# Samsung/iac

Measured on AMD Instinct MI355X. Metric: Msamples/s rendered (3rd-order HOA->binaural, 48 kHz), higher is better.
Workload: dtype f32

## Files before the change

### iac_amd/csrc/iamf_render.hip

```cpp
#include <hip/hip_runtime.h>

#include <math.h>
#include <stdint.h>
#include <atomic>
#include <stdio.h>
#include <stdlib.h>
#include <string.h>

#include <new>
#include <type_traits>
#include <vector>

#include "../../include/iamf_hip.h"

#define IAMF_FFT_HOST_TABLES

#include "render_entry.hpp"

namespace {

#include "render_common.hpp"
#include "render_downmix.hpp"
#include "render_fir.hpp"
#include "render_fir16.hpp"
// ... 46 lines not shown
};

extern "C" const uint8_t _binary_rdr_tables_bin_start[];
extern "C" const uint8_t _binary_rdr_tables_bin_end[];
extern "C" const uint8_t _binary_rdr_tables_tv_bin_start[];
extern "C" const uint8_t _binary_rdr_tables_tv_bin_end[];

struct Tables {
  int n = 0;
  const TableEntry *ents = nullptr;
  const float *data = nullptr;
  bool ok = false;
  explicit Tables(bool tv) {
    const uint8_t *b = tv ? _binary_rdr_tables_tv_bin_start : _binary_rdr_tables_bin_start;
    const size_t sz = tv ? (size_t)(_binary_rdr_tables_tv_bin_end - _binary_rdr_tables_tv_bin_start)
                         : (size_t)(_binary_rdr_tables_bin_end - _binary_rdr_tables_bin_start);
    if (sz < 12 || memcmp(b, "IARDRTB1", 8) != 0) return;
    uint32_t cnt;
    memcpy(&cnt, b + 8, 4);
    n = (int)cnt;
    ents = reinterpret_cast<const TableEntry *>(b + 12);
    data = reinterpret_cast<const float *>(b + 12 + sizeof(TableEntry) * cnt);
    ok = true;
  }
};

const Tables &tables(bool tv) {
  static Tables t(false), t_tv(true);
  return tv ? t_tv : t;
}

int find_matrix(int kind, int in_id, int out_id, iamf_hip_matrix *out, bool tv = false) {
  const Tables &t = tables(tv);
  if (!t.ok || !out) return -1;
  for (int i = 0; i < t.n; ++i) {
    const TableEntry &e = t.ents[i];
    if ((int)e.kind == kind && (int)e.in_id == in_id && (int)e.out_id == out_id) {
      out->kind = kind;
      out->in_id = in_id;
      out->out_id = out_id;
      out->channels = e.channels;
      out->lfe1 = e.lfe1;
      out->lfe2 = e.lfe2;
      out->m = e.m;
      out->n = e.n;
      out->mat = t.data + e.offset;
      return 0;
    }
  }
  return -1;
}

float ease(float x) {
  if (1.0 < x) return 1.0f;
  if (x < 0) return 0.0f;
  return 1.0f - powf(x - 1, 2.0);
}

}

struct iamf_hip_batch {
  iamf_hip_batch_config cfg;
  int device = 0;
  hipEvent_t done = nullptr;
  bool rendered = false;
  int m = 0, n_feeds = 0;
  int32_t src_feed[kMaxOut];
  uint32_t nz_mask[6] = {0, 0, 0, 0, 0, 0};
  int sparse = 0;
  int32_t *d_src_feed = nullptr;
  float thr = 0.f;
  int n_atk = 0, n_end = 0;
  std::vector<int64_t> spos;
  std::vector<uint8_t> sflushed;
  bool any_rendered = false;
  bool lp_scale_ok = false;
  float *d_matrix = nullptr, *d_gains = nullptr, *d_ctab = nullptr, *d_ring_y = nullptr,
        *d_ring_pm = nullptr;
  LimState *d_lim = nullptr;
  std::vector<float> h_gains;
  bool has2 = false;
  int m2 = 0;
  float *d_matrix2 = nullptr, *d_gains2 = nullptr;
  int32_t *d_src_feed2 = nullptr, *d_dmx_tab = nullptr;
  bool dmx = false;
  int dmx_n_in = 0, dmx_n_out = 0;
  float *d_pre = nullptr;
  int pre_l = 0;
  std::vector<float> h_fm;
  float *d_matrix_pre = nullptr;
  uint32_t nz_mask_pre[6] = {0, 0, 0, 0, 0, 0};
  int sparse_pre = 0;
  bool demix = false;
  int demix_steps = 0, demix_skip = 0, demix_layout = 0, demix_gmask = 0, demix_w4 = 0;
  int32_t *d_demix_tab = nullptr;
  float *d_demix_ftab = nullptr;
  bool fir = false;
  int fir_taps = 0;
  float *d_fir_hist[2] = {nullptr, nullptr};
  void *d_fir_h16 = nullptr;
  float *d_fir_pq = nullptr, *d_fir_tw = nullptr;
  float *d_fir_zero = nullptr;
  float *d_fir_pre[2] = {nullptr, nullptr};
  size_t fir_pre_bytes = 0;
  float *d_fir_y = nullptr;
  size_t fir_y_floats = 0;
  float *d_lp_in = nullptr;
  size_t lp_in_floats = 0;
  float *d_fir_id = nullptr;
  int32_t *d_fir_id_feed = nullptr;
  float fir_inv_scale = 1.f;
  int fir_cur = 0;
  bool lfe = false;
  float lfe_a1 = 0.f, lfe_a2 = 0.f, lfe_a3 = 0.f, lfe_b1 = 0.f, lfe_b2 = 0.f;
  double lfe_div = 0.0;
  float *d_lfe_state = nullptr, *d_lfe_next = nullptr, *d_lfe_u = nullptr;
  bool lfe_shared = false;
  size_t lfe_u_floats = 0;
  uint8_t *d_nat = nullptr;
  size_t nat_bytes = 0;
  uint8_t *d_dump = nullptr;
};

namespace {

bool on_batch_device(const iamf_hip_batch *b) {
  int dev = -1;
  return hipGetDevice(&dev) == hipSuccess && dev == b->device;
}

int quiesce(iamf_hip_batch *b) {
  if (b->rendered) HIPCHK(hipEventSynchronize(b->done));
  return IAMF_HIP_OK;
}

int reset_state(iamf_hip_batch *b) {
  const int ns = b->cfg.n_streams;
  std::vector<LimState> init((size_t)ns);
  for (auto &l : init) {
    l.g = 1.0f;
    l.gs = -1.0f;
    l.ge = -1.0f;
    l.n = b->n_end;
  }
  HIPCHK(hipMemcpy(b->d_lim, init.data(), sizeof(LimState) * ns, hipMemcpyHostToDevice));
  HIPCHK(hipMemset(b->d_ring_y, 0, sizeof(float) * (size_t)ns * b->cfg.out_channels * kSave));
  HIPCHK(hipMemset(b->d_ring_pm, 0, sizeof(float) * (size_t)ns * kSave));
  if (b->fir) {
    const size_t hb = sizeof(float) * (size_t)ns * b->m * 256;
    HIPCHK(hipMemset(b->d_fir_hist[0], 0, hb));
    HIPCHK(hipMemset(b->d_fir_hist[1], 0, hb));
    for (float *q : b->d_fir_pre)
      if (q) HIPCHK(hipMemset(q, 0, b->fir_pre_bytes));
  }
  if (b->lfe && !b->lfe_shared) {
    HIPCHK(hipMemset(b->d_lfe_state, 0, sizeof(float) * 4 * (size_t)ns));
    HIPCHK(hipMemset(b->d_lfe_next, 0, sizeof(float) * 2 * (size_t)ns));
  }
  b->spos.assign((size_t)ns, 0);
  b->sflushed.assign((size_t)ns, 0);
  b->any_rendered = false;
  return IAMF_HIP_OK;
}

template <int M>
void launch_m(const RenderParams &p, dim3 grid, size_t lds_bytes, hipStream_t st) {
  hipLaunchKernelGGL(render_kernel<M>, grid, dim3(kChunk), lds_bytes, st, p);
}

template <int M>
void launch_nolim_m(const RenderParams &p, hipStream_t st) {
  const int bytes = p.out_format == IAMF_HIP_FMT_S16 ? 2 : (p.out_format == IAMF_HIP_FMT_S24 ? 3 : 4);
  dim3 grid((unsigned)p.n_launch, (unsigned)((p.total + kNlChunk - 1) / kNlChunk));
  hipLaunchKernelGGL(render_nolim_kernel<M>, grid, dim3(256), (size_t)kNlChunk * p.out_ch * bytes, st, p);
}

template <int M, int OC>
void launch_fast_mc(const RenderParams &p, bool mixing, dim3 grid, hipStream_t st) {
  const size_t lds = sizeof(float) * (size_t)fast_lds_floats(OC, M);
  if (mixing) launch_big_lds<&render_fast_kernel<M, OC, 0, false, true>, 80 * 1024>(grid, dim3(256), lds, st, p);
  else launch_big_lds<&render_fast_kernel<M, OC>, 80 * 1024>(grid, dim3(256), lds, st, p);
}
template <int M>
void launch_fast_m(const RenderParams &p, bool mixing, dim3 grid, hipStream_t st) {
  if (p.out_ch == 1) launch_fast_mc<M, 1>(p, mixing, grid, st);
  else launch_fast_mc<M, 2>(p, mixing, grid, st);
}

template <int M, int OC>
void launch_fast_down_mc(const RenderParams &p, dim3 grid, hipStream_t st) {
  const size_t lds = sizeof(float) * (size_t)fast_lds_floats(OC, M);
  launch_big_lds<&render_fast_kernel<M, OC, 0, true>, 80 * 1024>(grid, dim3(256), lds, st, p);
}

template <int M>
void launch_wide_m(const RenderParams &p, dim3 grid, hipStream_t st) {
  const size_t lds = sizeof(float) * (size_t)wide_lds_floats(p.out_ch, M);
  if (p.use_mfma) launch_big_lds<&render_wide_kernel<M, true>, 80 * 1024>(grid, dim3(256), lds, st, p);
  else launch_big_lds<&render_wide_kernel<M, false>, 80 * 1024>(grid, dim3(256), lds, st, p);
}

int launch(const RenderParams &p, int m, size_t lds_bytes, hipStream_t st) {
  const Route r = pick_route(p, m);
  const dim3 grid((unsigned)p.n_launch);
  bool launched = false;
  switch (r.family) {
    case Family::Refused: return r.err;
    case Family::Lpcm: launched = iamf_hip_fast_lpcm_launch(&p, m, r.variant, st); break;
    case Family::FirSplit: {
      if (!dispatch(FirHomeM{}, m, [&](auto M) { launch_fft_m<M.value>(p, st); }) && !iamf_hip_fir_m2b_launch_fft(&p, m, st))
        return IAMF_HIP_ERR_INTERNAL;
      HIPCHK(hipGetLastError());
      RenderParams q = p;
      q.in = p.fir_y;
      q.in_stream_stride = 2 * (int64_t)p.total;
      q.in_frame_stride = 2 * (int64_t)p.total;
      q.frame_size = p.total;
      q.matrix = p.fir_id_matrix;
      q.src_feed = p.fir_id_feed;
      q.n_feeds = 2;
      q.fir_taps = 0;
      q.fir_hist = q.fir_hist_next = nullptr;
      launch_fast_m<2>(q, false, grid, st);
      launched = true;
      break;
    }
    case Family::FirFused:
      launched = dispatch(FirHomeM{}, m, [&](auto M) { launch_fir_m<M.value>(p, r.variant, st); }) ||
                 iamf_hip_fir_m2b_launch(&p, m, r.variant, st);
      break;
    case Family::FastDown:
      launched = dispatch(FastDownMC{}, mc(m, p.out_ch), [&](auto V) { launch_fast_down_mc<mc_m(V.value), mc_c(V.value)>(p, grid, st); });
      break;
    case Family::Wide4Lfe: launched = iamf_hip_wide4_lfe_launch(&p, m, st); break;
    case Family::Wide4Mix: launched = iamf_hip_wide4_mix_launch(&p, m, st); break;
    case Family::Wide4:
    case Family::Wide4Demix:
    case Family::Wide4Down: launched = iamf_hip_wide4_launch(&p, m, st); break;
    case Family::Nolim: launched = dispatch(NolimM{}, m, [&](auto M) { launch_nolim_m<M.value>(p, st); }); break;
    case Family::Fast: launched = dispatch(FastM{}, m, [&](auto M) { launch_fast_m<M.value>(p, r.variant != 0, grid, st); }); break;
    case Family::Wide: launched = dispatch(WideM{}, m, [&](auto M) { launch_wide_m<M.value>(p, grid, st); }); break;
    case Family::Generic: launched = dispatch(GenericM{}, m, [&](auto M) { launch_m<M.value>(p, grid, lds_bytes, st); }); break;
  }
  if (!launched) return IAMF_HIP_ERR_INTERNAL;
  HIPCHK(hipGetLastError());
  const RouteKey k = route_key(r, p, m);
  iamf_hip_route_count(k.family, k.variant, k.m, k.c, k.k);
  if (r.family == Family::FirSplit) iamf_hip_route_count(IAMF_HIP_ROUTE_FAST, 0, 2, 2, 0);
  return IAMF_HIP_OK;
}

const int kLayoutCount[9] = {1, 2, 6, 8, 10, 8, 10, 12, 6};
const int kLayoutCh[9][12] = {
    {kChMono},
    {kChL2, kChR2},
    {kChL7, kChR7, kChC, kChLFE, kChSL5, kChSR5},
    {kChL7, kChR7, kChC, kChLFE, kChSL5, kChSR5, kChHL, kChHR},
    {kChL7, kChR7, kChC, kChLFE, kChSL5, kChSR5, kChHFL, kChHFR, kChHBL, kChHBR},
    {kChL7, kChR7, kChC, kChLFE, kChSL7, kChSR7, kChBL7, kChBR7},
    {kChL7, kChR7, kChC, kChLFE, kChSL7, kChSR7, kChBL7, kChBR7, kChHL, kChHR},
    {kChL7, kChR7, kChC, kChLFE, kChSL7, kChSR7, kChBL7, kChBR7, kChHFL, kChHFR, kChHBL, kChHBR},
    {kChL3, kChR3, kChC, kChLFE, kChTL, kChTR},
};
const int kLayoutSurround[9] = {1, 2, 5, 5, 5, 7, 7, 7, 3};
const int kLayoutTop[9] = {0, 0, 0, 2, 4, 0, 2, 4, 2};

struct LpcmIn {
  const uint8_t *raw;
  int64_t stream_stride, frame_stride;
  int32_t off[16];
};
constexpr int kNotFused = INT32_MIN;

int lfe_prepass(iamf_hip_batch *b, const float *d_in, int64_t in_stream_stride, int64_t in_frame_stride, int ltotal,
                hipStream_t st, int s0, int cnt, int *t4_out) {
  const int ns = b->cfg.n_streams, nb = (ns + 63) / 64, t4 = (ltotal + 3) / 4;
  const size_t need_u = (size_t)nb * t4 * 64 * 4;
  if (need_u > b->lfe_u_floats) {
    HIPCHK(hipStreamSynchronize(st));
    (void)hipFree(b->d_lfe_u);
    b->d_lfe_u = nullptr;
    b->lfe_u_floats = 0;
    HIPCHK(hipMalloc(&b->d_lfe_u, sizeof(float) * need_u));
    b->lfe_u_floats = need_u;
  }
  LfeParams lp;
  memset(&lp, 0, sizeof(lp));
  lp.in = d_in;
  lp.in_stream_stride = in_stream_stride;
  lp.in_frame_stride = in_frame_stride;
  lp.pre_matrix = b->d_pre;
  lp.pre_l = b->pre_l;
  lp.pre_m = b->m;
  lp.frame_size = b->cfg.frame_size;
  lp.n_streams = ns;
  lp.total = ltotal;
  lp.t4 = t4;
  lp.a1 = b->lfe_a1; lp.a2 = b->lfe_a2; lp.a3 = b->lfe_a3; lp.b1 = b->lfe_b1; lp.b2 = b->lfe_b2;
  lp.state = b->d_lfe_state;
  lp.state_next = b->d_lfe_next;
  lp.u_t = reinterpret_cast<float4 *>(b->d_lfe_u);
  lp.s_first = s0;
  lp.s_count = cnt;
  hipLaunchKernelGGL(lfe_ff_kernel, dim3((unsigned)((t4 + kLfeTileQ - 1) / kLfeTileQ), (unsigned)nb), dim3(256), 0, st, lp);
  hipLaunchKernelGGL(lfe_chain_kernel, dim3((unsigned)nb), dim3(64), 0, st, lp);
  HIPCHK(hipGetLastError());
  *t4_out = t4;
  return IAMF_HIP_OK;
}

struct PreparedCall {
  RenderParams p;
  iamf_hip_render_args a;
  int m_eff;
  size_t lds;
  bool restride;
  int sc, bps;
  int64_t pos;
  int total, s0, cnt;
};

int render_prepare(iamf_hip_batch *b, const iamf_hip_render_args &a, int total, int s0, int cnt, const LpcmIn *lp, PreparedCall &pc) {
  if (!on_batch_device(b)) return IAMF_HIP_ERR_INVALID_STATE;
  if (lp && (b->fir || b->lfe || b->d_pre || b->demix || b->dmx || b->has2 || a.d_element_ramp || a.d_element2_ramp ||
             a.d_output_ramp || !b->lp_scale_ok || getenv("IAMF_HIP_LPCM_UNFUSED")))
    return kNotFused;
  if (s0 < 0 || cnt <= 0 || s0 + cnt > b->cfg.n_streams) return IAMF_HIP_ERR_BAD_ARG;
  if (a.lfe_pre_samples < 0 || a.lfe_post_samples < 0 ||
      ((a.lfe_pre_samples || a.lfe_post_samples) &&
       (a.n_frames != 1 || (int64_t)a.lfe_pre_samples + total + a.lfe_post_samples > b->cfg.frame_size)))
    return IAMF_HIP_ERR_BAD_ARG;
  const int64_t pos = b->spos[(size_t)s0];
  for (int i = s0; i < s0 + cnt; ++i)
    if (b->spos[(size_t)i] != pos || b->sflushed[(size_t)i]) return IAMF_HIP_ERR_INVALID_STATE;
  const bool whole = s0 == 0 && cnt == b->cfg.n_streams;
  if (!whole && b->fir) return IAMF_HIP_ERR_UNIMPLEMENTED;
  RenderParams &p = pc.p;
  memset(&p, 0, sizeof(p));
  p.stream0 = s0;
  p.n_launch = cnt;
  p.in = a.d_in;
  p.in_stream_stride = a.in_stream_stride;
  p.in_frame_stride = a.in_frame_stride;
  p.pcm = static_cast<uint8_t *>(a.d_pcm);
  p.pcm_stream_stride = a.pcm_stream_stride_bytes;
  p.matrix = b->d_matrix;
  p.gains = b->d_gains;
  p.ctab = b->d_ctab;
  p.lim = b->d_lim;
  p.ring_y = b->d_ring_y;
  p.ring_pm = b->d_ring_pm;
  p.pos0 = pos;
  p.total = total;
  p.frame_size = b->cfg.frame_size;
  p.n_streams = b->cfg.n_streams;
  p.n_feeds = b->n_feeds;
  p.out_ch = b->cfg.out_channels;
  p.og_ch = (b->cfg.out_gain_channels > 0 && b->cfg.out_gain_channels < b->cfg.out_channels) ? b->cfg.out_gain_channels : b->cfg.out_channels;
  p.out_format = b->cfg.out_format;
  p.limiter_on = b->cfg.limiter_enable ? 1 : 0;
  p.loudness_on = b->cfg.loudness_enable ? 1 : 0;
  bool tolerance = false;
  {
    const int proj = b->cfg.projection;
    const char *env = getenv("IAMF_HIP_PROJECTION");
    bool mf = proj == IAMF_HIP_PROJ_MFMA || (proj == IAMF_HIP_PROJ_AUTO && b->cfg.matrix.kind == IAMF_HIP_KIND_H2M);
    if (env && !strcmp(env, "exact")) mf = false;
    if (env && !strcmp(env, "mfma")) mf = true;
    p.use_mfma = (mf && b->n_feeds <= 32) ? 1 : 0;
    tolerance = mf;
  }
  p.n_atk = b->n_atk;
  p.n_end = b->n_end;
  p.thr = b->thr;
  p.src_feed = b->d_src_feed;
  p.dump = b->d_dump;
  for (int g = 0; g < 6; ++g) p.nz_mask[g] = b->nz_mask[g];
  p.sparse = getenv("IAMF_HIP_DENSE") ? 0 : b->sparse;
  if (b->has2 && a.d_in2) {
    p.in2 = a.d_in2;
    p.in2_stream_stride = a.in2_stream_stride;
    p.in2_frame_stride = a.in2_frame_stride;
    p.matrix2 = b->d_matrix2;
    p.src_feed2 = b->d_src_feed2;
    p.gains2 = b->d_gains2;
    p.m2 = b->m2;
  }
  p.elem_ramp = a.d_element_ramp;
  p.elem2_ramp = a.d_element2_ramp;
  p.out_ramp = a.d_output_ramp;
  p.ramp_stream_stride = a.ramp_stream_stride;
  if (b->dmx) {
    p.dmx_on = 1;
    p.dmx_frames = a.d_in ? a.d_dmx_frames : nullptr;
    p.dmx_n_in = b->dmx_n_in;
    p.dmx_n_out = b->dmx_n_out;
    p.dmx_tab = b->d_dmx_tab;
    p.dmx_in_layout = b->cfg.matrix.in_id;
    p.dmx_out_layout = b->cfg.matrix.out_id;
  }
  int m_eff = b->m;
  if (b->d_pre && a.d_in) {
    const int l = b->pre_l;
    if (tolerance && b->d_matrix_pre && FastM::has(l) && !p.in2) {
      p.matrix = b->d_matrix_pre;
      for (int g = 0; g < 6; ++g) p.nz_mask[g] = b->nz_mask_pre[g];
      p.sparse = getenv("IAMF_HIP_DENSE") ? 0 : b->sparse_pre;
      m_eff = l;
    } else {
      p.pre_matrix = b->d_pre;
      p.pre_l = b->pre_l;
    }
  }
  if (b->demix && a.d_in) {
    p.demix_on = 1;
    p.demix_steps = b->demix_steps;
    p.demix_skip = b->demix_skip;
    p.demix_tab = b->d_demix_tab;
    p.demix_ftab = b->d_demix_ftab;
    p.demix_frames = a.d_demix_frames;
    p.demix_i0 = a.n_frames == 1 ? a.demix_sample0 : 0;
    p.demix_layout = b->demix_layout;
    p.demix_gmask = b->demix_gmask;
    p.demix_w4 = b->demix_w4;
  }
  if (lp) {
    p.lpcm = lp->raw;
    p.lpcm_stream_stride = lp->stream_stride;
    p.lpcm_frame_stride = lp->frame_stride;
    for (int m = 0; m < 16; ++m) p.lpcm_off[m] = lp->off[m];
    if (pick_route(p, m_eff).family != Family::Lpcm) return kNotFused;
  }
  if (b->fir) {
    p.fir_taps = b->fir_taps;
    p.fir_hist = b->d_fir_hist[b->fir_cur];
    p.fir_hist_next = b->d_fir_hist[b->fir_cur ^ 1];
    p.fir_h16 = b->d_fir_h16;
    p.fir_inv_scale = b->fir_inv_scale;
    p.fir_pq = b->d_fir_pq;
    p.fir_tw = b->d_fir_tw;
    p.fir_zero = b->d_fir_zero;
    p.fir_pre = b->d_fir_pre[b->fir_cur];
    p.fir_pre_next = b->d_fir_pre[b->fir_cur ^ 1];
    if (a.d_in && b->d_fir_pq && (b->cfg.frame_size & 63) == 0 && !getenv("IAMF_HIP_FIR_FUSED") && !getenv("IAMF_HIP_FIR_F16") &&
        !getenv("IAMF_HIP_FIR_F32")) {
      const size_t need = (size_t)b->cfg.n_streams * 2 * (size_t)total;
      if (need > b->fir_y_floats) {
        HIPCHK(hipStreamSynchronize(static_cast<hipStream_t>(a.stream)));
        (void)hipFree(b->d_fir_y);
        b->d_fir_y = nullptr;
        b->fir_y_floats = 0;
        HIPCHK(hipMalloc(&b->d_fir_y, sizeof(float) * need));
        b->fir_y_floats = need;
      }
      p.fir_y = b->d_fir_y;
      p.fir_id_matrix = b->d_fir_id;
      p.fir_id_feed = b->d_fir_id_feed;
    }
  }
  if (b->lfe && a.d_in && total > 0) {
    const int lpre = a.lfe_pre_samples, lpost = a.lfe_post_samples;
    int t4 = 0;
    const int rc = lfe_prepass(b, a.d_in - lpre, a.in_stream_stride, a.in_frame_stride, lpre + total + lpost,
                               static_cast<hipStream_t>(a.stream), s0, cnt, &t4);
    if (rc) return rc;
    p.lfe = b->d_lfe_u;
    p.lfe_t4 = t4;
    p.lfe_k0 = lpre;
    p.lfe_div = b->lfe_div;
    for (int c = 0; c < b->cfg.out_channels && c < 32; ++c)
      if (b->src_feed[c] == -2) p.lfe_mask |= 1 << c;
  }
  const size_t lds = sizeof(float) * ((size_t)(p.out_ch + 2) * kRing + 3 * kChunk + kHead + 4 +
                                      ((b->dmx || b->demix) ? (size_t)kChCount * kChunk : 0));
  const int sc = b->cfg.pcm_stride_channels;
  const bool restride = sc > 0 && sc != p.out_ch;
  const int bps = iamf_hip_format_bytes(p.out_format);
  if (restride) {
    const size_t per_stream = (size_t)(total > kDelay ? total : kDelay) * p.out_ch * bps;
    const size_t need = per_stream * (size_t)p.n_streams;
    if (need > b->nat_bytes) {
      HIPCHK(hipStreamSynchronize(static_cast<hipStream_t>(a.stream)));
      (void)hipFree(b->d_nat);
      b->d_nat = nullptr;
      b->nat_bytes = 0;
      HIPCHK(hipMalloc(&b->d_nat, need));
      b->nat_bytes = need;
    }
    p.pcm = b->d_nat;
    p.pcm_stream_stride = (int64_t)per_stream;
  }
  pc.a = a;
  pc.m_eff = m_eff;
  pc.lds = lds;
  pc.restride = restride;
  pc.sc = sc;
  pc.bps = bps;
  pc.pos = pos;
  pc.total = total;
  pc.s0 = s0;
  pc.cnt = cnt;
  return IAMF_HIP_OK;
}

int render_launch(const PreparedCall &pc) {
  return launch(pc.p, pc.m_eff, pc.lds, static_cast<hipStream_t>(pc.a.stream));
}

int render_commit(iamf_hip_batch *b, const PreparedCall &pc) {
  const RenderParams &p = pc.p;
  const iamf_hip_render_args &a = pc.a;
  const bool restride = pc.restride;
  const int sc = pc.sc, bps = pc.bps, total = pc.total, s0 = pc.s0, cnt = pc.cnt;
  const int64_t pos = pc.pos;
  if (b->fir && p.in) b->fir_cur ^= 1;
  const int64_t before = p.limiter_on ? (pos > kDelay ? pos - kDelay : 0) : pos;
  for (int i = s0; i < s0 + cnt; ++i) b->spos[(size_t)i] = pos + total;
  b->any_rendered = true;
  const int64_t after = p.limiter_on ? (pos + total > kDelay ? pos + total - kDelay : 0) : pos + total;
  const int n_emit = (int)(after - before);
  if (restride && n_emit > 0) {
    const int64_t n_out = (int64_t)n_emit * sc + (p.out_ch > sc ? p.out_ch - sc : 0);
    hipLaunchKernelGGL(restride_kernel, dim3((unsigned)((n_out + 255) / 256), (unsigned)cnt), dim3(256), 0,
                       static_cast<hipStream_t>(a.stream), b->d_nat, p.pcm_stream_stride,
                       static_cast<uint8_t *>(a.d_pcm), a.pcm_stream_stride_bytes, n_emit, p.out_ch, sc, bps, s0);
    HIPCHK(hipGetLastError());
  }
  HIPCHK(hipEventRecord(b->done, static_cast<hipStream_t>(a.stream)));
  b->rendered = true;
  return n_emit;
}

int render_call(iamf_hip_batch *b, const iamf_hip_render_args &a, int total, int s0, int cnt, const LpcmIn *lp = nullptr) {
  PreparedCall pc;
  int r = render_prepare(b, a, total, s0, cnt, lp, pc);
  if (r != IAMF_HIP_OK) return r;
  r = render_launch(pc);
  if (r != IAMF_HIP_OK) return r;
  return render_commit(b, pc);
}

void build_feed_map(const iamf_hip_matrix &mx, int out_channels, std::vector<float> &fm, int32_t *src_feed) {
  for (int i = 0; i < kMaxOut; ++i) src_feed[i] = -1;
  for (int i = 0; i < mx.n; ++i) {
    int d = i;
    if (mx.kind == IAMF_HIP_KIND_H2M && (mx.lfe1 >= 0 || mx.lfe2 >= 0)) {
      if (mx.lfe1 >= 0 && mx.lfe1 <= i) ++d;
      if (mx.lfe2 >= 0 && mx.lfe2 <= i) ++d;
    }
    if (d < out_channels) src_feed[d] = i;
  }
  if (mx.kind == IAMF_HIP_KIND_H2M) {
    if (mx.lfe1 >= 0 && mx.lfe1 < out_channels) src_feed[mx.lfe1] = -1;
    if (mx.lfe2 >= 0 && mx.lfe2 < out_channels) src_feed[mx.lfe2] = -1;
  }
  fm.assign((size_t)mx.m * mx.n, 0.f);
  for (int f = 0; f < mx.n; ++f)
    for (int k = 0; k < mx.m; ++k)
      fm[(size_t)f * mx.m + k] = mx.kind == IAMF_HIP_KIND_H2M ? mx.mat[f * mx.m + k] : mx.mat[k * mx.n + f];
}

}

extern "C" {

int iamf_hip_get_h2m_matrix(int order, int out_id, iamf_hip_matrix *out) {
  return find_matrix(IAMF_HIP_KIND_H2M, order, out_id, out);
}

int iamf_hip_get_m2m_matrix(int in_id, int out_id, iamf_hip_matrix *out) {
  return find_matrix(IAMF_HIP_KIND_M2M, in_id, out_id, out);
}

int iamf_hip_get_m2m_matrix_variant(int variant, int in_id, int out_id, iamf_hip_matrix *out) {
  if (variant != IAMF_HIP_VARIANT_DEFAULT && variant != IAMF_HIP_VARIANT_SAMSUNG_TV) return -1;
  return find_matrix(IAMF_HIP_KIND_M2M, in_id, out_id, out, variant == IAMF_HIP_VARIANT_SAMSUNG_TV);
}

int iamf_hip_layout_channels(int out_id) {
  switch (out_id) {
    case IAMF_HIP_SS_A: return 2;
    case IAMF_HIP_SS_B: return 6;
    case IAMF_HIP_SS_C: return 8;
    case IAMF_HIP_SS_D: return 10;
    case IAMF_HIP_SS_E: return 11;
    case IAMF_HIP_SS_F: return 12;
    case IAMF_HIP_SS_G: return 14;
    case IAMF_HIP_SS_H: return 24;
    case IAMF_HIP_SS_I: return 8;
    case IAMF_HIP_SS_J: return 12;
    case IAMF_HIP_L_712: return 10;
    case IAMF_HIP_L_312: return 6;
    case IAMF_HIP_L_MONO: return 1;
    case IAMF_HIP_L_BINAURAL: return 2;
    default: return 0;
  }
}

int iamf_hip_format_bytes(int f) {
  switch (f) {
    case IAMF_HIP_FMT_S16: return 2;
    case IAMF_HIP_FMT_S24: return 3;
    case IAMF_HIP_FMT_S32: return 4;
    case IAMF_HIP_FMT_F32: return 4;
    default: return 0;
  }
}

// ... 1280 lines not shown
```

### iac_amd/csrc/lfe_chain_asm.inc

```
#define IAMF_LFE_RING 32
#define IAMF_LFE_ASM_BODY \
  "s_mov_b64 s[40:41], %[base]\n\t" \
  "s_mov_b32 s44, %[nrot]\n\t" \
  "v_mov_b32 v0, %[voff]\n\t" \
  "v_mov_b32 v2, %[b1]\n\t" \
  "v_mov_b32 v3, %[b2]\n\t" \
  "v_mov_b32 v12, 0x80000000\n\t" \
  "v_mov_b32 v13, 0x80000000\n\t" \
  "v_mul_f32 v10, v2, %[y1]\n\t" \
  "v_mul_f32 v11, v3, %[y1]\n\t" \
  "v_mul_f32 v9, v3, %[y2]\n\t" \
  "s_add_u32 s46, s40, 4096\n\t" \
  "s_addc_u32 s47, s41, 0\n\t" \
  "global_load_dwordx4 v[16:19], v0, s[46:47] offset:-4096\n\t" \
  "global_load_dwordx4 v[20:23], v0, s[46:47] offset:-3072\n\t" \
  "global_load_dwordx4 v[24:27], v0, s[46:47] offset:-2048\n\t" \
  "global_load_dwordx4 v[28:31], v0, s[46:47] offset:-1024\n\t" \
  "global_load_dwordx4 v[32:35], v0, s[46:47] offset:0\n\t" \
  "global_load_dwordx4 v[36:39], v0, s[46:47] offset:1024\n\t" \
  "global_load_dwordx4 v[40:43], v0, s[46:47] offset:2048\n\t" \
  "global_load_dwordx4 v[44:47], v0, s[46:47] offset:3072\n\t" \
  "s_add_u32 s46, s46, 8192\n\t" \
  "s_addc_u32 s47, s47, 0\n\t" \
  "global_load_dwordx4 v[48:51], v0, s[46:47] offset:-4096\n\t" \
  "global_load_dwordx4 v[52:55], v0, s[46:47] offset:-3072\n\t" \
  "global_load_dwordx4 v[56:59], v0, s[46:47] offset:-2048\n\t" \
  "global_load_dwordx4 v[60:63], v0, s[46:47] offset:-1024\n\t" \
  "global_load_dwordx4 v[64:67], v0, s[46:47] offset:0\n\t" \
  "global_load_dwordx4 v[68:71], v0, s[46:47] offset:1024\n\t" \
  "global_load_dwordx4 v[72:75], v0, s[46:47] offset:2048\n\t" \
  "global_load_dwordx4 v[76:79], v0, s[46:47] offset:3072\n\t" \
  "s_add_u32 s46, s46, 8192\n\t" \
  "s_addc_u32 s47, s47, 0\n\t" \
  "global_load_dwordx4 v[80:83], v0, s[46:47] offset:-4096\n\t" \
  "global_load_dwordx4 v[84:87], v0, s[46:47] offset:-3072\n\t" \
  "global_load_dwordx4 v[88:91], v0, s[46:47] offset:-2048\n\t" \
  "global_load_dwordx4 v[92:95], v0, s[46:47] offset:-1024\n\t" \
  "global_load_dwordx4 v[96:99], v0, s[46:47] offset:0\n\t" \
  "global_load_dwordx4 v[100:103], v0, s[46:47] offset:1024\n\t" \
  "global_load_dwordx4 v[104:107], v0, s[46:47] offset:2048\n\t" \
  "global_load_dwordx4 v[108:111], v0, s[46:47] offset:3072\n\t" \
  "s_add_u32 s46, s46, 8192\n\t" \
  "s_addc_u32 s47, s47, 0\n\t" \
  "global_load_dwordx4 v[112:115], v0, s[46:47] offset:-4096\n\t" \
  "global_load_dwordx4 v[116:119], v0, s[46:47] offset:-3072\n\t" \
  "global_load_dwordx4 v[120:123], v0, s[46:47] offset:-2048\n\t" \
  "global_load_dwordx4 v[124:127], v0, s[46:47] offset:-1024\n\t" \
  "global_load_dwordx4 v[128:131], v0, s[46:47] offset:0\n\t" \
  "global_load_dwordx4 v[132:135], v0, s[46:47] offset:1024\n\t" \
  "global_load_dwordx4 v[136:139], v0, s[46:47] offset:2048\n\t" \
  "global_load_dwordx4 v[140:143], v0, s[46:47] offset:3072\n\t" \
  "s_add_u32 s46, s46, 8192\n\t" \
  "s_addc_u32 s47, s47, 0\n\t" \
  "s_waitcnt vmcnt(0)\n\t" \
  "Llfe_rot%=:\n\t" \
  "s_sub_u32 s44, s44, 1\n\t" \
  "s_cmp_lg_u32 s44, 0\n\t" \
  "s_cselect_b32 s45, 32768, 0\n\t" \
  "s_add_u32 s42, s40, 4096\n\t" \
  "s_addc_u32 s43, s41, 0\n\t" \
  "s_add_u32 s46, s42, s45\n\t" \
  "s_addc_u32 s47, s43, 0\n\t" \
  "s_waitcnt vmcnt(56)\n\t" \
  "v_sub_f32 v16, v16, v10\n\t" \
  "v_sub_f32 v16, v16, v9\n\t" \
  "v_pk_mul_f32 v[4:5], v[16:17], v[2:3] op_sel:[0,0] op_sel_hi:[0,1]\n\t" \
  "v_sub_f32 v17, v17, v4\n\t" \
  "v_sub_f32 v17, v17, v11\n\t" \
  "v_pk_mul_f32 v[6:7], v[16:17], v[2:3] op_sel:[1,0] op_sel_hi:[1,1]\n\t" \
  "v_sub_f32 v18, v18, v6\n\t" \
  "v_sub_f32 v18, v18, v5\n\t" \
  "v_pk_mul_f32 v[8:9], v[18:19], v[2:3] op_sel:[0,0] op_sel_hi:[0,1]\n\t" \
  "v_sub_f32 v19, v19, v8\n\t" \
  "v_sub_f32 v19, v19, v7\n\t" \
  "v_pk_mul_f32 v[10:11], v[18:19], v[2:3] op_sel:[1,0] op_sel_hi:[1,1]\n\t" \
  "global_store_dwordx4 v0, v[16:19], s[42:43] offset:-4096\n\t" \
  "global_load_dwordx4 v[16:19], v0, s[46:47] offset:-4096\n\t" \
  "v_sub_f32 v20, v20, v10\n\t" \
  "v_sub_f32 v20, v20, v9\n\t" \
  "v_pk_mul_f32 v[4:5], v[20:21], v[2:3] op_sel:[0,0] op_sel_hi:[0,1]\n\t" \
  "v_sub_f32 v21, v21, v4\n\t" \
  "v_sub_f32 v21, v21, v11\n\t" \
  "v_pk_mul_f32 v[6:7], v[20:21], v[2:3] op_sel:[1,0] op_sel_hi:[1,1]\n\t" \
  "v_sub_f32 v22, v22, v6\n\t" \
  "v_sub_f32 v22, v22, v5\n\t" \
  "v_pk_mul_f32 v[8:9], v[22:23], v[2:3] op_sel:[0,0] op_sel_hi:[0,1]\n\t" \
  "v_sub_f32 v23, v23, v8\n\t" \
  "v_sub_f32 v23, v23, v7\n\t" \
  "v_pk_mul_f32 v[10:11], v[22:23], v[2:3] op_sel:[1,0] op_sel_hi:[1,1]\n\t" \
  "global_store_dwordx4 v0, v[20:23], s[42:43] offset:-3072\n\t" \
  "global_load_dwordx4 v[20:23], v0, s[46:47] offset:-3072\n\t" \
  "v_sub_f32 v24, v24, v10\n\t" \
  "v_sub_f32 v24, v24, v9\n\t" \
  "v_pk_mul_f32 v[4:5], v[24:25], v[2:3] op_sel:[0,0] op_sel_hi:[0,1]\n\t" \
  "v_sub_f32 v25, v25, v4\n\t" \
  "v_sub_f32 v25, v25, v11\n\t" \
  "v_pk_mul_f32 v[6:7], v[24:25], v[2:3] op_sel:[1,0] op_sel_hi:[1,1]\n\t" \
  "v_sub_f32 v26, v26, v6\n\t" \
  "v_sub_f32 v26, v26, v5\n\t" \
  "v_pk_mul_f32 v[8:9], v[26:27], v[2:3] op_sel:[0,0] op_sel_hi:[0,1]\n\t" \
  "v_sub_f32 v27, v27, v8\n\t" \
  "v_sub_f32 v27, v27, v7\n\t" \
  "v_pk_mul_f32 v[10:11], v[26:27], v[2:3] op_sel:[1,0] op_sel_hi:[1,1]\n\t" \
  "global_store_dwordx4 v0, v[24:27], s[42:43] offset:-2048\n\t" \
  "global_load_dwordx4 v[24:27], v0, s[46:47] offset:-2048\n\t" \
  "v_sub_f32 v28, v28, v10\n\t" \
  "v_sub_f32 v28, v28, v9\n\t" \
  "v_pk_mul_f32 v[4:5], v[28:29], v[2:3] op_sel:[0,0] op_sel_hi:[0,1]\n\t" \
  "v_sub_f32 v29, v29, v4\n\t" \
  "v_sub_f32 v29, v29, v11\n\t" \
  "v_pk_mul_f32 v[6:7], v[28:29], v[2:3] op_sel:[1,0] op_sel_hi:[1,1]\n\t" \
  "v_sub_f32 v30, v30, v6\n\t" \
  "v_sub_f32 v30, v30, v5\n\t" \
  "v_pk_mul_f32 v[8:9], v[30:31], v[2:3] op_sel:[0,0] op_sel_hi:[0,1]\n\t" \
  "v_sub_f32 v31, v31, v8\n\t" \
  "v_sub_f32 v31, v31, v7\n\t" \
  "v_pk_mul_f32 v[10:11], v[30:31], v[2:3] op_sel:[1,0] op_sel_hi:[1,1]\n\t" \
  "global_store_dwordx4 v0, v[28:31], s[42:43] offset:-1024\n\t" \
  "global_load_dwordx4 v[28:31], v0, s[46:47] offset:-1024\n\t" \
  "s_waitcnt vmcnt(56)\n\t" \
  "v_sub_f32 v32, v32, v10\n\t" \
  "v_sub_f32 v32, v32, v9\n\t" \
  "v_pk_mul_f32 v[4:5], v[32:33], v[2:3] op_sel:[0,0] op_sel_hi:[0,1]\n\t" \
  "v_sub_f32 v33, v33, v4\n\t" \
  "v_sub_f32 v33, v33, v11\n\t" \
  "v_pk_mul_f32 v[6:7], v[32:33], v[2:3] op_sel:[1,0] op_sel_hi:[1,1]\n\t" \
  "v_sub_f32 v34, v34, v6\n\t" \
  "v_sub_f32 v34, v34, v5\n\t" \
  "v_pk_mul_f32 v[8:9], v[34:35], v[2:3] op_sel:[0,0] op_sel_hi:[0,1]\n\t" \
  "v_sub_f32 v35, v35, v8\n\t" \
  "v_sub_f32 v35, v35, v7\n\t" \
  "v_pk_mul_f32 v[10:11], v[34:35], v[2:3] op_sel:[1,0] op_sel_hi:[1,1]\n\t" \
  "global_store_dwordx4 v0, v[32:35], s[42:43] offset:0\n\t" \
  "global_load_dwordx4 v[32:35], v0, s[46:47] offset:0\n\t" \
  "v_sub_f32 v36, v36, v10\n\t" \
  "v_sub_f32 v36, v36, v9\n\t" \
  "v_pk_mul_f32 v[4:5], v[36:37], v[2:3] op_sel:[0,0] op_sel_hi:[0,1]\n\t" \
  "v_sub_f32 v37, v37, v4\n\t" \
  "v_sub_f32 v37, v37, v11\n\t" \
  "v_pk_mul_f32 v[6:7], v[36:37], v[2:3] op_sel:[1,0] op_sel_hi:[1,1]\n\t" \
  "v_sub_f32 v38, v38, v6\n\t" \
  "v_sub_f32 v38, v38, v5\n\t" \
  "v_pk_mul_f32 v[8:9], v[38:39], v[2:3] op_sel:[0,0] op_sel_hi:[0,1]\n\t" \
  "v_sub_f32 v39, v39, v8\n\t" \
  "v_sub_f32 v39, v39, v7\n\t" \
  "v_pk_mul_f32 v[10:11], v[38:39], v[2:3] op_sel:[1,0] op_sel_hi:[1,1]\n\t" \
  "global_store_dwordx4 v0, v[36:39], s[42:43] offset:1024\n\t" \
  "global_load_dwordx4 v[36:39], v0, s[46:47] offset:1024\n\t" \
  "v_sub_f32 v40, v40, v10\n\t" \
  "v_sub_f32 v40, v40, v9\n\t" \
  "v_pk_mul_f32 v[4:5], v[40:41], v[2:3] op_sel:[0,0] op_sel_hi:[0,1]\n\t" \
  "v_sub_f32 v41, v41, v4\n\t" \
  "v_sub_f32 v41, v41, v11\n\t" \
  "v_pk_mul_f32 v[6:7], v[40:41], v[2:3] op_sel:[1,0] op_sel_hi:[1,1]\n\t" \
  "v_sub_f32 v42, v42, v6\n\t" \
  "v_sub_f32 v42, v42, v5\n\t" \
  "v_pk_mul_f32 v[8:9], v[42:43], v[2:3] op_sel:[0,0] op_sel_hi:[0,1]\n\t" \
  "v_sub_f32 v43, v43, v8\n\t" \
  "v_sub_f32 v43, v43, v7\n\t" \
  "v_pk_mul_f32 v[10:11], v[42:43], v[2:3] op_sel:[1,0] op_sel_hi:[1,1]\n\t" \
  "global_store_dwordx4 v0, v[40:43], s[42:43] offset:2048\n\t" \
  "global_load_dwordx4 v[40:43], v0, s[46:47] offset:2048\n\t" \
  "v_sub_f32 v44, v44, v10\n\t" \
  "v_sub_f32 v44, v44, v9\n\t" \
  "v_pk_mul_f32 v[4:5], v[44:45], v[2:3] op_sel:[0,0] op_sel_hi:[0,1]\n\t" \
  "v_sub_f32 v45, v45, v4\n\t" \
  "v_sub_f32 v45, v45, v11\n\t" \
  "v_pk_mul_f32 v[6:7], v[44:45], v[2:3] op_sel:[1,0] op_sel_hi:[1,1]\n\t" \
  "v_sub_f32 v46, v46, v6\n\t" \
  "v_sub_f32 v46, v46, v5\n\t" \
  "v_pk_mul_f32 v[8:9], v[46:47], v[2:3] op_sel:[0,0] op_sel_hi:[0,1]\n\t" \
  "v_sub_f32 v47, v47, v8\n\t" \
  "v_sub_f32 v47, v47, v7\n\t" \
  "v_pk_mul_f32 v[10:11], v[46:47], v[2:3] op_sel:[1,0] op_sel_hi:[1,1]\n\t" \
  "global_store_dwordx4 v0, v[44:47], s[42:43] offset:3072\n\t" \
  "global_load_dwordx4 v[44:47], v0, s[46:47] offset:3072\n\t" \
  "s_add_u32 s42, s42, 8192\n\t" \
  "s_addc_u32 s43, s43, 0\n\t" \
  "s_add_u32 s46, s46, 8192\n\t" \
  "s_addc_u32 s47, s47, 0\n\t" \
  "s_waitcnt vmcnt(56)\n\t" \
  "v_sub_f32 v48, v48, v10\n\t" \
  "v_sub_f32 v48, v48, v9\n\t" \
  "v_pk_mul_f32 v[4:5], v[48:49], v[2:3] op_sel:[0,0] op_sel_hi:[0,1]\n\t" \
  "v_sub_f32 v49, v49, v4\n\t" \
  "v_sub_f32 v49, v49, v11\n\t" \
  "v_pk_mul_f32 v[6:7], v[48:49], v[2:3] op_sel:[1,0] op_sel_hi:[1,1]\n\t" \
  "v_sub_f32 v50, v50, v6\n\t" \
  "v_sub_f32 v50, v50, v5\n\t" \
  "v_pk_mul_f32 v[8:9], v[50:51], v[2:3] op_sel:[0,0] op_sel_hi:[0,1]\n\t" \
  "v_sub_f32 v51, v51, v8\n\t" \
  "v_sub_f32 v51, v51, v7\n\t" \
  "v_pk_mul_f32 v[10:11], v[50:51], v[2:3] op_sel:[1,0] op_sel_hi:[1,1]\n\t" \
  "global_store_dwordx4 v0, v[48:51], s[42:43] offset:-4096\n\t" \
  "global_load_dwordx4 v[48:51], v0, s[46:47] offset:-4096\n\t" \
  "v_sub_f32 v52, v52, v10\n\t" \
  "v_sub_f32 v52, v52, v9\n\t" \
  "v_pk_mul_f32 v[4:5], v[52:53], v[2:3] op_sel:[0,0] op_sel_hi:[0,1]\n\t" \
  "v_sub_f32 v53, v53, v4\n\t" \
  "v_sub_f32 v53, v53, v11\n\t" \
  "v_pk_mul_f32 v[6:7], v[52:53], v[2:3] op_sel:[1,0] op_sel_hi:[1,1]\n\t" \
  "v_sub_f32 v54, v54, v6\n\t" \
  "v_sub_f32 v54, v54, v5\n\t" \
  "v_pk_mul_f32 v[8:9], v[54:55], v[2:3] op_sel:[0,0] op_sel_hi:[0,1]\n\t" \
  "v_sub_f32 v55, v55, v8\n\t" \
  "v_sub_f32 v55, v55, v7\n\t" \
  "v_pk_mul_f32 v[10:11], v[54:55], v[2:3] op_sel:[1,0] op_sel_hi:[1,1]\n\t" \
  "global_store_dwordx4 v0, v[52:55], s[42:43] offset:-3072\n\t" \
  "global_load_dwordx4 v[52:55], v0, s[46:47] offset:-3072\n\t" \
  "v_sub_f32 v56, v56, v10\n\t" \
  "v_sub_f32 v56, v56, v9\n\t" \
  "v_pk_mul_f32 v[4:5], v[56:57], v[2:3] op_sel:[0,0] op_sel_hi:[0,1]\n\t" \
  "v_sub_f32 v57, v57, v4\n\t" \
  "v_sub_f32 v57, v57, v11\n\t" \
  "v_pk_mul_f32 v[6:7], v[56:57], v[2:3] op_sel:[1,0] op_sel_hi:[1,1]\n\t" \
  "v_sub_f32 v58, v58, v6\n\t" \
  "v_sub_f32 v58, v58, v5\n\t" \
  "v_pk_mul_f32 v[8:9], v[58:59], v[2:3] op_sel:[0,0] op_sel_hi:[0,1]\n\t" \
  "v_sub_f32 v59, v59, v8\n\t" \
  "v_sub_f32 v59, v59, v7\n\t" \
  "v_pk_mul_f32 v[10:11], v[58:59], v[2:3] op_sel:[1,0] op_sel_hi:[1,1]\n\t" \
  "global_store_dwordx4 v0, v[56:59], s[42:43] offset:-2048\n\t" \
  "global_load_dwordx4 v[56:59], v0, s[46:47] offset:-2048\n\t" \
  "v_sub_f32 v60, v60, v10\n\t" \
  "v_sub_f32 v60, v60, v9\n\t" \
  "v_pk_mul_f32 v[4:5], v[60:61], v[2:3] op_sel:[0,0] op_sel_hi:[0,1]\n\t" \
  "v_sub_f32 v61, v61, v4\n\t" \
  "v_sub_f32 v61, v61, v11\n\t" \
  "v_pk_mul_f32 v[6:7], v[60:61], v[2:3] op_sel:[1,0] op_sel_hi:[1,1]\n\t" \
  "v_sub_f32 v62, v62, v6\n\t" \
  "v_sub_f32 v62, v62, v5\n\t" \
  "v_pk_mul_f32 v[8:9], v[62:63], v[2:3] op_sel:[0,0] op_sel_hi:[0,1]\n\t" \
  "v_sub_f32 v63, v63, v8\n\t" \
  "v_sub_f32 v63, v63, v7\n\t" \
  "v_pk_mul_f32 v[10:11], v[62:63], v[2:3] op_sel:[1,0] op_sel_hi:[1,1]\n\t" \
  "global_store_dwordx4 v0, v[60:63], s[42:43] offset:-1024\n\t" \
  "global_load_dwordx4 v[60:63], v0, s[46:47] offset:-1024\n\t" \
  "s_waitcnt vmcnt(56)\n\t" \
  "v_sub_f32 v64, v64, v10\n\t" \
  "v_sub_f32 v64, v64, v9\n\t" \
  "v_pk_mul_f32 v[4:5], v[64:65], v[2:3] op_sel:[0,0] op_sel_hi:[0,1]\n\t" \
  "v_sub_f32 v65, v65, v4\n\t" \
  "v_sub_f32 v65, v65, v11\n\t" \
  "v_pk_mul_f32 v[6:7], v[64:65], v[2:3] op_sel:[1,0] op_sel_hi:[1,1]\n\t" \
  "v_sub_f32 v66, v66, v6\n\t" \
  "v_sub_f32 v66, v66, v5\n\t" \
  "v_pk_mul_f32 v[8:9], v[66:67], v[2:3] op_sel:[0,0] op_sel_hi:[0,1]\n\t" \
  "v_sub_f32 v67, v67, v8\n\t" \
  "v_sub_f32 v67, v67, v7\n\t" \
  "v_pk_mul_f32 v[10:11], v[66:67], v[2:3] op_sel:[1,0] op_sel_hi:[1,1]\n\t" \
  "global_store_dwordx4 v0, v[64:67], s[42:43] offset:0\n\t" \
  "global_load_dwordx4 v[64:67], v0, s[46:47] offset:0\n\t" \
  "v_sub_f32 v68, v68, v10\n\t" \
  "v_sub_f32 v68, v68, v9\n\t" \
  "v_pk_mul_f32 v[4:5], v[68:69], v[2:3] op_sel:[0,0] op_sel_hi:[0,1]\n\t" \
  "v_sub_f32 v69, v69, v4\n\t" \
  "v_sub_f32 v69, v69, v11\n\t" \
  "v_pk_mul_f32 v[6:7], v[68:69], v[2:3] op_sel:[1,0] op_sel_hi:[1,1]\n\t" \
  "v_sub_f32 v70, v70, v6\n\t" \
  "v_sub_f32 v70, v70, v5\n\t" \
  "v_pk_mul_f32 v[8:9], v[70:71], v[2:3] op_sel:[0,0] op_sel_hi:[0,1]\n\t" \
  "v_sub_f32 v71, v71, v8\n\t" \
  "v_sub_f32 v71, v71, v7\n\t" \
  "v_pk_mul_f32 v[10:11], v[70:71], v[2:3] op_sel:[1,0] op_sel_hi:[1,1]\n\t" \
  "global_store_dwordx4 v0, v[68:71], s[42:43] offset:1024\n\t" \
  "global_load_dwordx4 v[68:71], v0, s[46:47] offset:1024\n\t" \
  "v_sub_f32 v72, v72, v10\n\t" \
  "v_sub_f32 v72, v72, v9\n\t" \
  "v_pk_mul_f32 v[4:5], v[72:73], v[2:3] op_sel:[0,0] op_sel_hi:[0,1]\n\t" \
  "v_sub_f32 v73, v73, v4\n\t" \
  "v_sub_f32 v73, v73, v11\n\t" \
  "v_pk_mul_f32 v[6:7], v[72:73], v[2:3] op_sel:[1,0] op_sel_hi:[1,1]\n\t" \
  "v_sub_f32 v74, v74, v6\n\t" \
  "v_sub_f32 v74, v74, v5\n\t" \
  "v_pk_mul_f32 v[8:9], v[74:75], v[2:3] op_sel:[0,0] op_sel_hi:[0,1]\n\t" \
  "v_sub_f32 v75, v75, v8\n\t" \
  "v_sub_f32 v75, v75, v7\n\t" \
  "v_pk_mul_f32 v[10:11], v[74:75], v[2:3] op_sel:[1,0] op_sel_hi:[1,1]\n\t" \
  "global_store_dwordx4 v0, v[72:75], s[42:43] offset:2048\n\t" \
  "global_load_dwordx4 v[72:75], v0, s[46:47] offset:2048\n\t" \
  "v_sub_f32 v76, v76, v10\n\t" \
  "v_sub_f32 v76, v76, v9\n\t" \
  "v_pk_mul_f32 v[4:5], v[76:77], v[2:3] op_sel:[0,0] op_sel_hi:[0,1]\n\t" \
  "v_sub_f32 v77, v77, v4\n\t" \
  "v_sub_f32 v77, v77, v11\n\t" \
  "v_pk_mul_f32 v[6:7], v[76:77], v[2:3] op_sel:[1,0] op_sel_hi:[1,1]\n\t" \
  "v_sub_f32 v78, v78, v6\n\t" \
  "v_sub_f32 v78, v78, v5\n\t" \
  "v_pk_mul_f32 v[8:9], v[78:79], v[2:3] op_sel:[0,0] op_sel_hi:[0,1]\n\t" \
  "v_sub_f32 v79, v79, v8\n\t" \
  "v_sub_f32 v79, v79, v7\n\t" \
  "v_pk_mul_f32 v[10:11], v[78:79], v[2:3] op_sel:[1,0] op_sel_hi:[1,1]\n\t" \
  "global_store_dwordx4 v0, v[76:79], s[42:43] offset:3072\n\t" \
  "global_load_dwordx4 v[76:79], v0, s[46:47] offset:3072\n\t" \
  "s_add_u32 s42, s42, 8192\n\t" \
  "s_addc_u32 s43, s43, 0\n\t" \
  "s_add_u32 s46, s46, 8192\n\t" \
  "s_addc_u32 s47, s47, 0\n\t" \
  "s_waitcnt vmcnt(56)\n\t" \
  "v_sub_f32 v80, v80, v10\n\t" \
  "v_sub_f32 v80, v80, v9\n\t" \
  "v_pk_mul_f32 v[4:5], v[80:81], v[2:3] op_sel:[0,0] op_sel_hi:[0,1]\n\t" \
  "v_sub_f32 v81, v81, v4\n\t" \
  "v_sub_f32 v81, v81, v11\n\t" \
  "v_pk_mul_f32 v[6:7], v[80:81], v[2:3] op_sel:[1,0] op_sel_hi:[1,1]\n\t" \
  "v_sub_f32 v82, v82, v6\n\t" \
  "v_sub_f32 v82, v82, v5\n\t" \
  "v_pk_mul_f32 v[8:9], v[82:83], v[2:3] op_sel:[0,0] op_sel_hi:[0,1]\n\t" \
  "v_sub_f32 v83, v83, v8\n\t" \
  "v_sub_f32 v83, v83, v7\n\t" \
  "v_pk_mul_f32 v[10:11], v[82:83], v[2:3] op_sel:[1,0] op_sel_hi:[1,1]\n\t" \
  "global_store_dwordx4 v0, v[80:83], s[42:43] offset:-4096\n\t" \
  "global_load_dwordx4 v[80:83], v0, s[46:47] offset:-4096\n\t" \
  "v_sub_f32 v84, v84, v10\n\t" \
  "v_sub_f32 v84, v84, v9\n\t" \
  "v_pk_mul_f32 v[4:5], v[84:85], v[2:3] op_sel:[0,0] op_sel_hi:[0,1]\n\t" \
  "v_sub_f32 v85, v85, v4\n\t" \
  "v_sub_f32 v85, v85, v11\n\t" \
  "v_pk_mul_f32 v[6:7], v[84:85], v[2:3] op_sel:[1,0] op_sel_hi:[1,1]\n\t" \
  "v_sub_f32 v86, v86, v6\n\t" \
  "v_sub_f32 v86, v86, v5\n\t" \
  "v_pk_mul_f32 v[8:9], v[86:87], v[2:3] op_sel:[0,0] op_sel_hi:[0,1]\n\t" \
  "v_sub_f32 v87, v87, v8\n\t" \
  "v_sub_f32 v87, v87, v7\n\t" \
  "v_pk_mul_f32 v[10:11], v[86:87], v[2:3] op_sel:[1,0] op_sel_hi:[1,1]\n\t" \
  "global_store_dwordx4 v0, v[84:87], s[42:43] offset:-3072\n\t" \
  "global_load_dwordx4 v[84:87], v0, s[46:47] offset:-3072\n\t" \
  "v_sub_f32 v88, v88, v10\n\t" \
  "v_sub_f32 v88, v88, v9\n\t" \
  "v_pk_mul_f32 v[4:5], v[88:89], v[2:3] op_sel:[0,0] op_sel_hi:[0,1]\n\t" \
  "v_sub_f32 v89, v89, v4\n\t" \
  "v_sub_f32 v89, v89, v11\n\t" \
  "v_pk_mul_f32 v[6:7], v[88:89], v[2:3] op_sel:[1,0] op_sel_hi:[1,1]\n\t" \
  "v_sub_f32 v90, v90, v6\n\t" \
  "v_sub_f32 v90, v90, v5\n\t" \
  "v_pk_mul_f32 v[8:9], v[90:91], v[2:3] op_sel:[0,0] op_sel_hi:[0,1]\n\t" \
  "v_sub_f32 v91, v91, v8\n\t" \
  "v_sub_f32 v91, v91, v7\n\t" \
  "v_pk_mul_f32 v[10:11], v[90:91], v[2:3] op_sel:[1,0] op_sel_hi:[1,1]\n\t" \
  "global_store_dwordx4 v0, v[88:91], s[42:43] offset:-2048\n\t" \
  "global_load_dwordx4 v[88:91], v0, s[46:47] offset:-2048\n\t" \
  "v_sub_f32 v92, v92, v10\n\t" \
  "v_sub_f32 v92, v92, v9\n\t" \
  "v_pk_mul_f32 v[4:5], v[92:93], v[2:3] op_sel:[0,0] op_sel_hi:[0,1]\n\t" \
  "v_sub_f32 v93, v93, v4\n\t" \
  "v_sub_f32 v93, v93, v11\n\t" \
  "v_pk_mul_f32 v[6:7], v[92:93], v[2:3] op_sel:[1,0] op_sel_hi:[1,1]\n\t" \
  "v_sub_f32 v94, v94, v6\n\t" \
  "v_sub_f32 v94, v94, v5\n\t" \
  "v_pk_mul_f32 v[8:9], v[94:95], v[2:3] op_sel:[0,0] op_sel_hi:[0,1]\n\t" \
  "v_sub_f32 v95, v95, v8\n\t" \
  "v_sub_f32 v95, v95, v7\n\t" \
  "v_pk_mul_f32 v[10:11], v[94:95], v[2:3] op_sel:[1,0] op_sel_hi:[1,1]\n\t" \
  "global_store_dwordx4 v0, v[92:95], s[42:43] offset:-1024\n\t" \
  "global_load_dwordx4 v[92:95], v0, s[46:47] offset:-1024\n\t" \
  "s_waitcnt vmcnt(56)\n\t" \
  "v_sub_f32 v96, v96, v10\n\t" \
  "v_sub_f32 v96, v96, v9\n\t" \
  "v_pk_mul_f32 v[4:5], v[96:97], v[2:3] op_sel:[0,0] op_sel_hi:[0,1]\n\t" \
  "v_sub_f32 v97, v97, v4\n\t" \
  "v_sub_f32 v97, v97, v11\n\t" \
  "v_pk_mul_f32 v[6:7], v[96:97], v[2:3] op_sel:[1,0] op_sel_hi:[1,1]\n\t" \
  "v_sub_f32 v98, v98, v6\n\t" \
  "v_sub_f32 v98, v98, v5\n\t" \
  "v_pk_mul_f32 v[8:9], v[98:99], v[2:3] op_sel:[0,0] op_sel_hi:[0,1]\n\t" \
  "v_sub_f32 v99, v99, v8\n\t" \
  "v_sub_f32 v99, v99, v7\n\t" \
  "v_pk_mul_f32 v[10:11], v[98:99], v[2:3] op_sel:[1,0] op_sel_hi:[1,1]\n\t" \
  "global_store_dwordx4 v0, v[96:99], s[42:43] offset:0\n\t" \
  "global_load_dwordx4 v[96:99], v0, s[46:47] offset:0\n\t" \
  "v_sub_f32 v100, v100, v10\n\t" \
  "v_sub_f32 v100, v100, v9\n\t" \
  "v_pk_mul_f32 v[4:5], v[100:101], v[2:3] op_sel:[0,0] op_sel_hi:[0,1]\n\t" \
  "v_sub_f32 v101, v101, v4\n\t" \
  "v_sub_f32 v101, v101, v11\n\t" \
  "v_pk_mul_f32 v[6:7], v[100:101], v[2:3] op_sel:[1,0] op_sel_hi:[1,1]\n\t" \
  "v_sub_f32 v102, v102, v6\n\t" \
  "v_sub_f32 v102, v102, v5\n\t" \
  "v_pk_mul_f32 v[8:9], v[102:103], v[2:3] op_sel:[0,0] op_sel_hi:[0,1]\n\t" \
  "v_sub_f32 v103, v103, v8\n\t" \
  "v_sub_f32 v103, v103, v7\n\t" \
  "v_pk_mul_f32 v[10:11], v[102:103], v[2:3] op_sel:[1,0] op_sel_hi:[1,1]\n\t" \
  "global_store_dwordx4 v0, v[100:103], s[42:43] offset:1024\n\t" \
  "global_load_dwordx4 v[100:103], v0, s[46:47] offset:1024\n\t" \
  "v_sub_f32 v104, v104, v10\n\t" \
  "v_sub_f32 v104, v104, v9\n\t" \
  "v_pk_mul_f32 v[4:5], v[104:105], v[2:3] op_sel:[0,0] op_sel_hi:[0,1]\n\t" \
  "v_sub_f32 v105, v105, v4\n\t" \
  "v_sub_f32 v105, v105, v11\n\t" \
  "v_pk_mul_f32 v[6:7], v[104:105], v[2:3] op_sel:[1,0] op_sel_hi:[1,1]\n\t" \
  "v_sub_f32 v106, v106, v6\n\t" \
  "v_sub_f32 v106, v106, v5\n\t" \
  "v_pk_mul_f32 v[8:9], v[106:107], v[2:3] op_sel:[0,0] op_sel_hi:[0,1]\n\t" \
  "v_sub_f32 v107, v107, v8\n\t" \
  "v_sub_f32 v107, v107, v7\n\t" \
  "v_pk_mul_f32 v[10:11], v[106:107], v[2:3] op_sel:[1,0] op_sel_hi:[1,1]\n\t" \
  "global_store_dwordx4 v0, v[104:107], s[42:43] offset:2048\n\t" \
  "global_load_dwordx4 v[104:107], v0, s[46:47] offset:2048\n\t" \
  "v_sub_f32 v108, v108, v10\n\t" \
  "v_sub_f32 v108, v108, v9\n\t" \
  "v_pk_mul_f32 v[4:5], v[108:109], v[2:3] op_sel:[0,0] op_sel_hi:[0,1]\n\t" \
  "v_sub_f32 v109, v109, v4\n\t" \
  "v_sub_f32 v109, v109, v11\n\t" \
  "v_pk_mul_f32 v[6:7], v[108:109], v[2:3] op_sel:[1,0] op_sel_hi:[1,1]\n\t" \
  "v_sub_f32 v110, v110, v6\n\t" \
  "v_sub_f32 v110, v110, v5\n\t" \
  "v_pk_mul_f32 v[8:9], v[110:111], v[2:3] op_sel:[0,0] op_sel_hi:[0,1]\n\t" \
  "v_sub_f32 v111, v111, v8\n\t" \
  "v_sub_f32 v111, v111, v7\n\t" \
  "v_pk_mul_f32 v[10:11], v[110:111], v[2:3] op_sel:[1,0] op_sel_hi:[1,1]\n\t" \
  "global_store_dwordx4 v0, v[108:111], s[42:43] offset:3072\n\t" \
  "global_load_dwordx4 v[108:111], v0, s[46:47] offset:3072\n\t" \
  "s_add_u32 s42, s42, 8192\n\t" \
  "s_addc_u32 s43, s43, 0\n\t" \
  "s_add_u32 s46, s46, 8192\n\t" \
  "s_addc_u32 s47, s47, 0\n\t" \
  "s_waitcnt vmcnt(56)\n\t" \
  "v_sub_f32 v112, v112, v10\n\t" \
  "v_sub_f32 v112, v112, v9\n\t" \
  "v_pk_mul_f32 v[4:5], v[112:113], v[2:3] op_sel:[0,0] op_sel_hi:[0,1]\n\t" \
  "v_sub_f32 v113, v113, v4\n\t" \
  "v_sub_f32 v113, v113, v11\n\t" \
  "v_pk_mul_f32 v[6:7], v[112:113], v[2:3] op_sel:[1,0] op_sel_hi:[1,1]\n\t" \
  "v_sub_f32 v114, v114, v6\n\t" \
  "v_sub_f32 v114, v114, v5\n\t" \
  "v_pk_mul_f32 v[8:9], v[114:115], v[2:3] op_sel:[0,0] op_sel_hi:[0,1]\n\t" \
  "v_sub_f32 v115, v115, v8\n\t" \
  "v_sub_f32 v115, v115, v7\n\t" \
  "v_pk_mul_f32 v[10:11], v[114:115], v[2:3] op_sel:[1,0] op_sel_hi:[1,1]\n\t" \
  "global_store_dwordx4 v0, v[112:115], s[42:43] offset:-4096\n\t" \
  "global_load_dwordx4 v[112:115], v0, s[46:47] offset:-4096\n\t" \
  "v_sub_f32 v116, v116, v10\n\t" \
  "v_sub_f32 v116, v116, v9\n\t" \
  "v_pk_mul_f32 v[4:5], v[116:117], v[2:3] op_sel:[0,0] op_sel_hi:[0,1]\n\t" \
  "v_sub_f32 v117, v117, v4\n\t" \
  "v_sub_f32 v117, v117, v11\n\t" \
  "v_pk_mul_f32 v[6:7], v[116:117], v[2:3] op_sel:[1,0] op_sel_hi:[1,1]\n\t" \
  "v_sub_f32 v118, v118, v6\n\t" \
  "v_sub_f32 v118, v118, v5\n\t" \
  "v_pk_mul_f32 v[8:9], v[118:119], v[2:3] op_sel:[0,0] op_sel_hi:[0,1]\n\t" \
  "v_sub_f32 v119, v119, v8\n\t" \
  "v_sub_f32 v119, v119, v7\n\t" \
  "v_pk_mul_f32 v[10:11], v[118:119], v[2:3] op_sel:[1,0] op_sel_hi:[1,1]\n\t" \
  "global_store_dwordx4 v0, v[116:119], s[42:43] offset:-3072\n\t" \
  "global_load_dwordx4 v[116:119], v0, s[46:47] offset:-3072\n\t" \
  "v_sub_f32 v120, v120, v10\n\t" \
  "v_sub_f32 v120, v120, v9\n\t" \
  "v_pk_mul_f32 v[4:5], v[120:121], v[2:3] op_sel:[0,0] op_sel_hi:[0,1]\n\t" \
  "v_sub_f32 v121, v121, v4\n\t" \
  "v_sub_f32 v121, v121, v11\n\t" \
  "v_pk_mul_f32 v[6:7], v[120:121], v[2:3] op_sel:[1,0] op_sel_hi:[1,1]\n\t" \
  "v_sub_f32 v122, v122, v6\n\t" \
  "v_sub_f32 v122, v122, v5\n\t" \
  "v_pk_mul_f32 v[8:9], v[122:123], v[2:3] op_sel:[0,0] op_sel_hi:[0,1]\n\t" \
  "v_sub_f32 v123, v123, v8\n\t" \
  "v_sub_f32 v123, v123, v7\n\t" \
  "v_pk_mul_f32 v[10:11], v[122:123], v[2:3] op_sel:[1,0] op_sel_hi:[1,1]\n\t" \
  "global_store_dwordx4 v0, v[120:123], s[42:43] offset:-2048\n\t" \
  "global_load_dwordx4 v[120:123], v0, s[46:47] offset:-2048\n\t" \
  "v_sub_f32 v124, v124, v10\n\t" \
  "v_sub_f32 v124, v124, v9\n\t" \
  "v_pk_mul_f32 v[4:5], v[124:125], v[2:3] op_sel:[0,0] op_sel_hi:[0,1]\n\t" \
  "v_sub_f32 v125, v125, v4\n\t" \
  "v_sub_f32 v125, v125, v11\n\t" \
  "v_pk_mul_f32 v[6:7], v[124:125], v[2:3] op_sel:[1,0] op_sel_hi:[1,1]\n\t" \
  "v_sub_f32 v126, v126, v6\n\t" \
  "v_sub_f32 v126, v126, v5\n\t" \
  "v_pk_mul_f32 v[8:9], v[126:127], v[2:3] op_sel:[0,0] op_sel_hi:[0,1]\n\t" \
  "v_sub_f32 v127, v127, v8\n\t" \
  "v_sub_f32 v127, v127, v7\n\t" \
  "v_pk_mul_f32 v[10:11], v[126:127], v[2:3] op_sel:[1,0] op_sel_hi:[1,1]\n\t" \
  "global_store_dwordx4 v0, v[124:127], s[42:43] offset:-1024\n\t" \
  "global_load_dwordx4 v[124:127], v0, s[46:47] offset:-1024\n\t" \
  "s_waitcnt vmcnt(56)\n\t" \
  "v_sub_f32 v128, v128, v10\n\t" \
  "v_sub_f32 v128, v128, v9\n\t" \
  "v_pk_mul_f32 v[4:5], v[128:129], v[2:3] op_sel:[0,0] op_sel_hi:[0,1]\n\t" \
  "v_sub_f32 v129, v129, v4\n\t" \
  "v_sub_f32 v129, v129, v11\n\t" \
  "v_pk_mul_f32 v[6:7], v[128:129], v[2:3] op_sel:[1,0] op_sel_hi:[1,1]\n\t" \
  "v_sub_f32 v130, v130, v6\n\t" \
  "v_sub_f32 v130, v130, v5\n\t" \
  "v_pk_mul_f32 v[8:9], v[130:131], v[2:3] op_sel:[0,0] op_sel_hi:[0,1]\n\t" \
  "v_sub_f32 v131, v131, v8\n\t" \
  "v_sub_f32 v131, v131, v7\n\t" \
  "v_pk_mul_f32 v[10:11], v[130:131], v[2:3] op_sel:[1,0] op_sel_hi:[1,1]\n\t" \
  "global_store_dwordx4 v0, v[128:131], s[42:43] offset:0\n\t" \
  "global_load_dwordx4 v[128:131], v0, s[46:47] offset:0\n\t" \
  "v_sub_f32 v132, v132, v10\n\t" \
  "v_sub_f32 v132, v132, v9\n\t" \
  "v_pk_mul_f32 v[4:5], v[132:133], v[2:3] op_sel:[0,0] op_sel_hi:[0,1]\n\t" \
  "v_sub_f32 v133, v133, v4\n\t" \
  "v_sub_f32 v133, v133, v11\n\t" \
  "v_pk_mul_f32 v[6:7], v[132:133], v[2:3] op_sel:[1,0] op_sel_hi:[1,1]\n\t" \
  "v_sub_f32 v134, v134, v6\n\t" \
  "v_sub_f32 v134, v134, v5\n\t" \
  "v_pk_mul_f32 v[8:9], v[134:135], v[2:3] op_sel:[0,0] op_sel_hi:[0,1]\n\t" \
  "v_sub_f32 v135, v135, v8\n\t" \
  "v_sub_f32 v135, v135, v7\n\t" \
  "v_pk_mul_f32 v[10:11], v[134:135], v[2:3] op_sel:[1,0] op_sel_hi:[1,1]\n\t" \
  "global_store_dwordx4 v0, v[132:135], s[42:43] offset:1024\n\t" \
  "global_load_dwordx4 v[132:135], v0, s[46:47] offset:1024\n\t" \
  "v_sub_f32 v136, v136, v10\n\t" \
  "v_sub_f32 v136, v136, v9\n\t" \
  "v_pk_mul_f32 v[4:5], v[136:137], v[2:3] op_sel:[0,0] op_sel_hi:[0,1]\n\t" \
  "v_sub_f32 v137, v137, v4\n\t" \
  "v_sub_f32 v137, v137, v11\n\t" \
  "v_pk_mul_f32 v[6:7], v[136:137], v[2:3] op_sel:[1,0] op_sel_hi:[1,1]\n\t" \
  "v_sub_f32 v138, v138, v6\n\t" \
  "v_sub_f32 v138, v138, v5\n\t" \
  "v_pk_mul_f32 v[8:9], v[138:139], v[2:3] op_sel:[0,0] op_sel_hi:[0,1]\n\t" \
  "v_sub_f32 v139, v139, v8\n\t" \
  "v_sub_f32 v139, v139, v7\n\t" \
  "v_pk_mul_f32 v[10:11], v[138:139], v[2:3] op_sel:[1,0] op_sel_hi:[1,1]\n\t" \
  "global_store_dwordx4 v0, v[136:139], s[42:43] offset:2048\n\t" \
  "global_load_dwordx4 v[136:139], v0, s[46:47] offset:2048\n\t" \
  "v_sub_f32 v140, v140, v10\n\t" \
  "v_sub_f32 v140, v140, v9\n\t" \
  "v_pk_mul_f32 v[4:5], v[140:141], v[2:3] op_sel:[0,0] op_sel_hi:[0,1]\n\t" \
  "v_sub_f32 v141, v141, v4\n\t" \
  "v_sub_f32 v141, v141, v11\n\t" \
  "v_pk_mul_f32 v[6:7], v[140:141], v[2:3] op_sel:[1,0] op_sel_hi:[1,1]\n\t" \
  "v_sub_f32 v142, v142, v6\n\t" \
  "v_sub_f32 v142, v142, v5\n\t" \
  "v_pk_mul_f32 v[8:9], v[142:143], v[2:3] op_sel:[0,0] op_sel_hi:[0,1]\n\t" \
  "v_sub_f32 v143, v143, v8\n\t" \
  "v_sub_f32 v143, v143, v7\n\t" \
  "v_pk_mul_f32 v[10:11], v[142:143], v[2:3] op_sel:[1,0] op_sel_hi:[1,1]\n\t" \
  "global_store_dwordx4 v0, v[140:143], s[42:43] offset:3072\n\t" \
  "global_load_dwordx4 v[140:143], v0, s[46:47] offset:3072\n\t" \
  "s_add_u32 s42, s42, 8192\n\t" \
  "s_addc_u32 s43, s43, 0\n\t" \
  "s_add_u32 s46, s46, 8192\n\t" \
  "s_addc_u32 s47, s47, 0\n\t" \
  "s_add_u32 s40, s40, 32768\n\t" \
  "s_addc_u32 s41, s41, 0\n\t" \
  "s_cmp_lg_u32 s44, 0\n\t" \
  "s_cbranch_scc1 Llfe_rot%=\n\t" \
  "s_waitcnt vmcnt(0)\n\t" \
  "v_mov_b32 %[y1], v143\n\t" \
  "v_mov_b32 %[y2], v142\n\t" \
  ""
#define IAMF_LFE_ASM_CLOBBERS \
  "v0", "v1", "v2", "v3", "v4", "v5", "v6", "v7", "v8", "v9", "v10", "v11", "v12", "v13", "v14", "v15", "v16", "v17", "v18", "v19", "v20", "v21", "v22", "v23", "v24", "v25", "v26", "v27", "v28", "v29", "v30", "v31", "v32", "v33", "v34", "v35", "v36", "v37", "v38", "v39", "v40", "v41", "v42", "v43", "v44", "v45", "v46", "v47", "v48", "v49", "v50", "v51", "v52", "v53", "v54", "v55", "v56", "v57", "v58", "v59", "v60", "v61", "v62", "v63", "v64", "v65", "v66", "v67", "v68", "v69", "v70", "v71", "v72", "v73", "v74", "v75", "v76", "v77", "v78", "v79", "v80", "v81", "v82", "v83", "v84", "v85", "v86", "v87", "v88", "v89", "v90", "v91", "v92", "v93", "v94", "v95", "v96", "v97", "v98", "v99", "v100", "v101", "v102", "v103", "v104", "v105", "v106", "v107", "v108", "v109", "v110", "v111", "v112", "v113", "v114", "v115", "v116", "v117", "v118", "v119", "v120", "v121", "v122", "v123", "v124", "v125", "v126", "v127", "v128", "v129", "v130", "v131", "v132", "v133", "v134", "v135", "v136", "v137", "v138", "v139", "v140", "v141", "v142", "v143", "s40", "s41", "s42", "s43", "s44", "s45", "s46", "s47", "scc", "memory"
```

### iac_amd/csrc/render_lfe.hpp

```cpp
#pragma once

#include "lfe_chain_asm.inc"

constexpr int kLfeTileQ = 16;

struct LfeParams {
  const float *in;
  int64_t in_stream_stride, in_frame_stride;
  const float *pre_matrix;
  int32_t pre_l, pre_m;
  int32_t frame_size, n_streams, total, t4;
  float a1, a2, a3, b1, b2;
  float *state;
  float *state_next;
  float4 *u_t;
  int32_t s_first, s_count;
};

__device__ __forceinline__ int64_t lfe_index(int s, int k, int t4) {
  return ((((int64_t)(s >> 6) * t4 + (k >> 2)) * 64 + (s & 63)) << 2) + (k & 3);
}

__device__ __forceinline__ float lfe_w_at(const LfeParams &p, int s, int k) {
  const int f = k / p.frame_size, i = k - f * p.frame_size;
  const float *src = p.in + (int64_t)s * p.in_stream_stride + (int64_t)f * p.in_frame_stride + i;
  if (!p.pre_matrix) return src[0];
  float w = 0.f;
  for (int l = 0; l < p.pre_l; ++l) w = w + src[(int64_t)l * p.frame_size] * p.pre_matrix[l * p.pre_m];
  return w;
}

__global__ __launch_bounds__(256) void lfe_ff_kernel(const LfeParams p) {
  __shared__ float4 tile[kLfeTileQ * 65];
  const int t = threadIdx.x;
  const int q_base = blockIdx.x * kLfeTileQ, sb = blockIdx.y;
#pragma unroll
  for (int pass = 0; pass < 4; ++pass) {
    const int q = t & 15, sl = (t >> 4) + 16 * pass;
    const int s = sb * 64 + sl, k0 = 4 * (q_base + q);
    float4 u = make_float4(0.f, 0.f, 0.f, 0.f);
    if (s >= p.s_first && s < p.s_first + p.s_count && k0 < p.total) {
      const float h1 = p.state[4 * s + 0], h2 = p.state[4 * s + 1];
      float wm1, wm2, w[4], uu[4];
      const bool quick = !p.pre_matrix && ((p.frame_size | p.in_stream_stride | p.in_frame_stride) & 3) == 0 &&
                         (reinterpret_cast<uintptr_t>(p.in) & 15) == 0 && k0 + 4 <= p.total;
      if (quick) {
        const int f = k0 / p.frame_size, i0 = k0 - f * p.frame_size;
        const float *src = p.in + (int64_t)s * p.in_stream_stride + (int64_t)f * p.in_frame_stride + i0;
        const float4 q = *reinterpret_cast<const float4 *>(src);
        w[0] = q.x, w[1] = q.y, w[2] = q.z, w[3] = q.w;
        if (i0 >= 4) {
          wm1 = src[-1];
          wm2 = src[-2];
        } else if (k0 == 0) {
          wm1 = h1;
          wm2 = h2;
        } else {
          const float *prv = p.in + (int64_t)s * p.in_stream_stride + (int64_t)(f - 1) * p.in_frame_stride + p.frame_size;
          wm1 = prv[-1];
          wm2 = prv[-2];
        }
      } else {
        wm1 = k0 >= 1 ? lfe_w_at(p, s, k0 - 1) : h1;
        wm2 = k0 >= 2 ? lfe_w_at(p, s, k0 - 2) : (k0 == 1 ? h1 : h2);
      }
#pragma unroll
      for (int i = 0; i < 4; ++i) {
        if (!quick) w[i] = k0 + i < p.total ? lfe_w_at(p, s, k0 + i) : 0.f;
        const float a = i >= 1 ? w[i - 1] : wm1, b = i >= 2 ? w[i - 2] : (i == 1 ? wm1 : wm2);
        uu[i] = (p.a1 * w[i] + p.a2 * a) + p.a3 * b;
      }
      u = make_float4(uu[0], uu[1], uu[2], uu[3]);
      if (k0 + 4 >= p.total) {
        const int il = p.total - 1 - k0;
        p.state_next[2 * s + 0] = w[il];
        p.state_next[2 * s + 1] = il >= 1 ? w[il - 1] : wm1;
      }
    }
    tile[q * 65 + sl] = u;
  }
  __syncthreads();
#pragma unroll
  for (int pass = 0; pass < 4; ++pass) {
    const int q = (t >> 6) + 4 * pass, sl = t & 63;
    if (q_base + q < p.t4) p.u_t[((int64_t)sb * p.t4 + q_base + q) * 64 + sl] = tile[q * 65 + sl];
  }
}

__global__ __launch_bounds__(64) void lfe_chain_kernel(const LfeParams p) {
  const int lane = threadIdx.x, sb = blockIdx.x;
  const int s = sb * 64 + lane;
  const bool active = s >= p.s_first && s < p.s_first + p.s_count;
  const int sc = active ? s : p.s_first;
  float y1 = p.state[4 * sc + 2], y2 = p.state[4 * sc + 3];
  const float b1 = p.b1, b2 = p.b2;
  float4 *row = p.u_t + (int64_t)sb * p.t4 * 64 + lane;
  const int nfull = p.total >> 2;
  auto step4 = [&](const float4 u) {
    float4 o;
    o.x = (u.x - b1 * y1) - b2 * y2;
    o.y = (u.y - b1 * o.x) - b2 * y1;
    o.z = (u.z - b1 * o.y) - b2 * o.x;
    o.w = (u.w - b1 * o.z) - b2 * o.y;
    y2 = o.z;
    y1 = o.w;
    return o;
  };
  int q_done = 0;
  {
    const int nrot = nfull / IAMF_LFE_RING;
    if (nrot > 0) {
      const float4 *base = p.u_t + (int64_t)sb * p.t4 * 64;
      const unsigned voff = (unsigned)lane * 16u;
      asm volatile(IAMF_LFE_ASM_BODY
                   : [y1] "+v"(y1), [y2] "+v"(y2)
                   : [base] "s"(base), [nrot] "s"(nrot), [voff] "v"(voff), [b1] "v"(b1), [b2] "v"(b2)
                   : IAMF_LFE_ASM_CLOBBERS);
      q_done = nrot * IAMF_LFE_RING;
    }
  }
  {
    const int nrem = nfull - q_done;
    float4 rem[IAMF_LFE_RING];
#pragma unroll
    for (int i = 0; i < IAMF_LFE_RING; ++i)
      if (i < nrem) rem[i] = row[(int64_t)(q_done + i) * 64];
#pragma unroll
    for (int i = 0; i < IAMF_LFE_RING; ++i)
      if (i < nrem) row[(int64_t)(q_done + i) * 64] = step4(rem[i]);
  }
  const int left = p.total - 4 * nfull;
  if (left > 0) {
    const float4 u = row[(int64_t)nfull * 64];
    float4 o;
    o.x = (u.x - b1 * y1) - b2 * y2;
    o.y = (u.y - b1 * o.x) - b2 * y1;
    o.z = (u.z - b1 * o.y) - b2 * o.x;
    o.w = 0.f;
    row[(int64_t)nfull * 64] = o;
    const float r1 = left == 3 ? o.z : (left == 2 ? o.y : o.x);
    const float r2 = left == 3 ? o.y : (left == 2 ? o.x : y1);
    y2 = r2;
    y1 = r1;
  }
  if (active) {
    p.state[4 * s + 0] = p.state_next[2 * s + 0];
    p.state[4 * s + 1] = p.state_next[2 * s + 1];
    p.state[4 * s + 2] = y1;
    p.state[4 * s + 3] = y2;
  }
}
```

Measured before the change: 87220.

## Fuse LFE feed-forward and IIR chain into one LDS-pipelined kernel

Merges the separate LFE feed-forward kernel and the recurrence chain kernel into a single kernel. Helper waves fetch input and compute the feed-forward terms into a triple-buffered LDS tile, while a chain wave runs the hand-written IIR recurrence out of LDS instead of global memory. This removes one kernel launch and the global round trip of the intermediate u buffer. In exchange it adds a __syncthreads per tile, uses fewer streams per block, and shrinks the asm ring to 16 entries.

```diff
diff --git a/iac_amd/csrc/iamf_render.hip b/iac_amd/csrc/iamf_render.hip
--- a/iac_amd/csrc/iamf_render.hip
+++ b/iac_amd/csrc/iamf_render.hip
@@ -372,8 +372,7 @@
   lp.u_t = reinterpret_cast<float4 *>(b->d_lfe_u);
   lp.s_first = s0;
   lp.s_count = cnt;
-  hipLaunchKernelGGL(lfe_ff_kernel, dim3((unsigned)((t4 + kLfeTileQ - 1) / kLfeTileQ), (unsigned)nb), dim3(256), 0, st, lp);
-  hipLaunchKernelGGL(lfe_chain_kernel, dim3((unsigned)nb), dim3(64), 0, st, lp);
+  hipLaunchKernelGGL(lfe_chain_kernel, dim3((unsigned)(nb * (64 / kLfeSW))), dim3(kLfeThreads), 0, st, lp);
   HIPCHK(hipGetLastError());
   *t4_out = t4;
   return IAMF_HIP_OK;
diff --git a/iac_amd/csrc/lfe_chain_asm.inc b/iac_amd/csrc/lfe_chain_asm.inc
--- a/iac_amd/csrc/lfe_chain_asm.inc
+++ b/iac_amd/csrc/lfe_chain_asm.inc
@@ -1,8 +1,8 @@
-#define IAMF_LFE_RING 32
+#define IAMF_LFE_RING 16
+#define IAMF_LFE_ROW_BYTES 272
 #define IAMF_LFE_ASM_BODY \
-  "s_mov_b64 s[40:41], %[base]\n\t" \
   "s_mov_b32 s44, %[nrot]\n\t" \
-  "v_mov_b32 v0, %[voff]\n\t" \
+  "v_mov_b32 v0, %[lds]\n\t" \
   "v_mov_b32 v2, %[b1]\n\t" \
   "v_mov_b32 v3, %[b2]\n\t" \
   "v_mov_b32 v12, 0x80000000\n\t" \
@@ -10,58 +10,21 @@
   "v_mul_f32 v10, v2, %[y1]\n\t" \
   "v_mul_f32 v11, v3, %[y1]\n\t" \
   "v_mul_f32 v9, v3, %[y2]\n\t" \
-  "s_add_u32 s46, s40, 4096\n\t" \
-  "s_addc_u32 s47, s41, 0\n\t" \
-  "global_load_dwordx4 v[16:19], v0, s[46:47] offset:-4096\n\t" \
-  "global_load_dwordx4 v[20:23], v0, s[46:47] offset:-3072\n\t" \
-  "global_load_dwordx4 v[24:27], v0, s[46:47] offset:-2048\n\t" \
-  "global_load_dwordx4 v[28:31], v0, s[46:47] offset:-1024\n\t" \
-  "global_load_dwordx4 v[32:35], v0, s[46:47] offset:0\n\t" \
-  "global_load_dwordx4 v[36:39], v0, s[46:47] offset:1024\n\t" \
-  "global_load_dwordx4 v[40:43], v0, s[46:47] offset:2048\n\t" \
-  "global_load_dwordx4 v[44:47], v0, s[46:47] offset:3072\n\t" \
-  "s_add_u32 s46, s46, 8192\n\t" \
-  "s_addc_u32 s47, s47, 0\n\t" \
-  "global_load_dwordx4 v[48:51], v0, s[46:47] offset:-4096\n\t" \
-  "global_load_dwordx4 v[52:55], v0, s[46:47] offset:-3072\n\t" \
-  "global_load_dwordx4 v[56:59], v0, s[46:47] offset:-2048\n\t" \
-  "global_load_dwordx4 v[60:63], v0, s[46:47] offset:-1024\n\t" \
-  "global_load_dwordx4 v[64:67], v0, s[46:47] offset:0\n\t" \
-  "global_load_dwordx4 v[68:71], v0, s[46:47] offset:1024\n\t" \
-  "global_load_dwordx4 v[72:75], v0, s[46:47] offset:2048\n\t" \
-  "global_load_dwordx4 v[76:79], v0, s[46:47] offset:3072\n\t" \
-  "s_add_u32 s46, s46, 8192\n\t" \
-  "s_addc_u32 s47, s47, 0\n\t" \
-  "global_load_dwordx4 v[80:83], v0, s[46:47] offset:-4096\n\t" \
-  "global_load_dwordx4 v[84:87], v0, s[46:47] offset:-3072\n\t" \
-  "global_load_dwordx4 v[88:91], v0, s[46:47] offset:-2048\n\t" \
-  "global_load_dwordx4 v[92:95], v0, s[46:47] offset:-1024\n\t" \
-  "global_load_dwordx4 v[96:99], v0, s[46:47] offset:0\n\t" \
-  "global_load_dwordx4 v[100:103], v0, s[46:47] offset:1024\n\t" \
-  "global_load_dwordx4 v[104:107], v0, s[46:47] offset:2048\n\t" \
-  "global_load_dwordx4 v[108:111], v0, s[46:47] offset:3072\n\t" \
-  "s_add_u32 s46, s46, 8192\n\t" \
-  "s_addc_u32 s47, s47, 0\n\t" \
-  "global_load_dwordx4 v[112:115], v0, s[46:47] offset:-4096\n\t" \
-  "global_load_dwordx4 v[116:119], v0, s[46:47] offset:-3072\n\t" \
-  "global_load_dwordx4 v[120:123], v0, s[46:47] offset:-2048\n\t" \
-  "global_load_dwordx4 v[124:127], v0, s[46:47] offset:-1024\n\t" \
-  "global_load_dwordx4 v[128:131], v0, s[46:47] offset:0\n\t" \
-  "global_load_dwordx4 v[132:135], v0, s[46:47] offset:1024\n\t" \
-  "global_load_dwordx4 v[136:139], v0, s[46:47] offset:2048\n\t" \
-  "global_load_dwordx4 v[140:143], v0, s[46:47] offset:3072\n\t" \
-  "s_add_u32 s46, s46, 8192\n\t" \
-  "s_addc_u32 s47, s47, 0\n\t" \
-  "s_waitcnt vmcnt(0)\n\t" \
+  "ds_read_b128 v[16:19], v0 offset:0\n\t" \
+  "ds_read_b128 v[20:23], v0 offset:272\n\t" \
+  "ds_read_b128 v[24:27], v0 offset:544\n\t" \
+  "ds_read_b128 v[28:31], v0 offset:816\n\t" \
+  "ds_read_b128 v[32:35], v0 offset:1088\n\t" \
+  "ds_read_b128 v[36:39], v0 offset:1360\n\t" \
+  "ds_read_b128 v[40:43], v0 offset:1632\n\t" \
+  "ds_read_b128 v[44:47], v0 offset:1904\n\t" \
+  "s_waitcnt lgkmcnt(0)\n\t" \
   "Llfe_rot%=:\n\t" \
   "s_sub_u32 s44, s44, 1\n\t" \
   "s_cmp_lg_u32 s44, 0\n\t" \
-  "s_cselect_b32 s45, 32768, 0\n\t" \
-  "s_add_u32 s42, s40, 4096\n\t" \
-  "s_addc_u32 s43, s41, 0\n\t" \
-  "s_add_u32 s46, s42, s45\n\t" \
-  "s_addc_u32 s47, s43, 0\n\t" \
-  "s_waitcnt vmcnt(56)\n\t" \
+  "s_cselect_b32 s45, 0, 2176\n\t" \
+  "v_subrev_u32 v1, s45, v0\n\t" \
+  "s_waitcnt lgkmcnt(8)\n\t" \
   "v_sub_f32 v16, v16, v10\n\t" \
   "v_sub_f32 v16, v16, v9\n\t" \
   "v_pk_mul_f32 v[4:5], v[16:17], v[2:3] op_sel:[0,0] op_sel_hi:[0,1]\n\t" \
@@ -74,8 +37,8 @@
   "v_sub_f32 v19, v19, v8\n\t" \
   "v_sub_f32 v19, v19, v7\n\t" \
   "v_pk_mul_f32 v[10:11], v[18:19], v[2:3] op_sel:[1,0] op_sel_hi:[1,1]\n\t" \
-  "global_store_dwordx4 v0, v[16:19], s[42:43] offset:-4096\n\t" \
-  "global_load_dwordx4 v[16:19], v0, s[46:47] offset:-4096\n\t" \
+  "ds_write_b128 v0, v[16:19] offset:0\n\t" \
+  "ds_read_b128 v[16:19], v0 offset:2176\n\t" \
   "v_sub_f32 v20, v20, v10\n\t" \
   "v_sub_f32 v20, v20, v9\n\t" \
   "v_pk_mul_f32 v[4:5], v[20:21], v[2:3] op_sel:[0,0] op_sel_hi:[0,1]\n\t" \
@@ -88,8 +51,8 @@
   "v_sub_f32 v23, v23, v8\n\t" \
   "v_sub_f32 v23, v23, v7\n\t" \
   "v_pk_mul_f32 v[10:11], v[22:23], v[2:3] op_sel:[1,0] op_sel_hi:[1,1]\n\t" \
-  "global_store_dwordx4 v0, v[20:23], s[42:43] offset:-3072\n\t" \
-  "global_load_dwordx4 v[20:23], v0, s[46:47] offset:-3072\n\t" \
+  "ds_write_b128 v0, v[20:23] offset:272\n\t" \
+  "ds_read_b128 v[20:23], v0 offset:2448\n\t" \
   "v_sub_f32 v24, v24, v10\n\t" \
   "v_sub_f32 v24, v24, v9\n\t" \
   "v_pk_mul_f32 v[4:5], v[24:25], v[2:3] op_sel:[0,0] op_sel_hi:[0,1]\n\t" \
@@ -102,8 +65,8 @@
   "v_sub_f32 v27, v27, v8\n\t" \
   "v_sub_f32 v27, v27, v7\n\t" \
   "v_pk_mul_f32 v[10:11], v[26:27], v[2:3] op_sel:[1,0] op_sel_hi:[1,1]\n\t" \
-  "global_store_dwordx4 v0, v[24:27], s[42:43] offset:-2048\n\t" \
-  "global_load_dwordx4 v[24:27], v0, s[46:47] offset:-2048\n\t" \
+  "ds_write_b128 v0, v[24:27] offset:544\n\t" \
+  "ds_read_b128 v[24:27], v0 offset:2720\n\t" \
   "v_sub_f32 v28, v28, v10\n\t" \
   "v_sub_f32 v28, v28, v9\n\t" \
   "v_pk_mul_f32 v[4:5], v[28:29], v[2:3] op_sel:[0,0] op_sel_hi:[0,1]\n\t" \
@@ -116,9 +79,9 @@
   "v_sub_f32 v31, v31, v8\n\t" \
   "v_sub_f32 v31, v31, v7\n\t" \
   "v_pk_mul_f32 v[10:11], v[30:31], v[2:3] op_sel:[1,0] op_sel_hi:[1,1]\n\t" \
-  "global_store_dwordx4 v0, v[28:31], s[42:43] offset:-1024\n\t" \
-  "global_load_dwordx4 v[28:31], v0, s[46:47] offset:-1024\n\t" \
-  "s_waitcnt vmcnt(56)\n\t" \
+  "ds_write_b128 v0, v[28:31] offset:816\n\t" \
+  "ds_read_b128 v[28:31], v0 offset:2992\n\t" \
+  "s_waitcnt lgkmcnt(8)\n\t" \
   "v_sub_f32 v32, v32, v10\n\t" \
   "v_sub_f32 v32, v32, v9\n\t" \
   "v_pk_mul_f32 v[4:5], v[32:33], v[2:3] op_sel:[0,0] op_sel_hi:[0,1]\n\t" \
@@ -131,8 +94,8 @@
   "v_sub_f32 v35, v35, v8\n\t" \
   "v_sub_f32 v35, v35, v7\n\t" \
   "v_pk_mul_f32 v[10:11], v[34:35], v[2:3] op_sel:[1,0] op_sel_hi:[1,1]\n\t" \
-  "global_store_dwordx4 v0, v[32:35], s[42:43] offset:0\n\t" \
-  "global_load_dwordx4 v[32:35], v0, s[46:47] offset:0\n\t" \
+  "ds_write_b128 v0, v[32:35] offset:1088\n\t" \
+  "ds_read_b128 v[32:35], v0 offset:3264\n\t" \
   "v_sub_f32 v36, v36, v10\n\t" \
   "v_sub_f32 v36, v36, v9\n\t" \
   "v_pk_mul_f32 v[4:5], v[36:37], v[2:3] op_sel:[0,0] op_sel_hi:[0,1]\n\t" \
@@ -145,8 +108,8 @@
   "v_sub_f32 v39, v39, v8\n\t" \
   "v_sub_f32 v39, v39, v7\n\t" \
   "v_pk_mul_f32 v[10:11], v[38:39], v[2:3] op_sel:[1,0] op_sel_hi:[1,1]\n\t" \
-  "global_store_dwordx4 v0, v[36:39], s[42:43] offset:1024\n\t" \
-  "global_load_dwordx4 v[36:39], v0, s[46:47] offset:1024\n\t" \
+  "ds_write_b128 v0, v[36:39] offset:1360\n\t" \
+  "ds_read_b128 v[36:39], v0 offset:3536\n\t" \
   "v_sub_f32 v40, v40, v10\n\t" \
   "v_sub_f32 v40, v40, v9\n\t" \
   "v_pk_mul_f32 v[4:5], v[40:41], v[2:3] op_sel:[0,0] op_sel_hi:[0,1]\n\t" \
@@ -159,8 +122,8 @@
   "v_sub_f32 v43, v43, v8\n\t" \
   "v_sub_f32 v43, v43, v7\n\t" \
   "v_pk_mul_f32 v[10:11], v[42:43], v[2:3] op_sel:[1,0] op_sel_hi:[1,1]\n\t" \
-  "global_store_dwordx4 v0, v[40:43], s[42:43] offset:2048\n\t" \
-  "global_load_dwordx4 v[40:43], v0, s[46:47] offset:2048\n\t" \
+  "ds_write_b128 v0, v[40:43] offset:1632\n\t" \
+  "ds_read_b128 v[40:43], v0 offset:3808\n\t" \
   "v_sub_f32 v44, v44, v10\n\t" \
   "v_sub_f32 v44, v44, v9\n\t" \
   "v_pk_mul_f32 v[4:5], v[44:45], v[2:3] op_sel:[0,0] op_sel_hi:[0,1]\n\t" \
@@ -173,373 +136,128 @@
   "v_sub_f32 v47, v47, v8\n\t" \
   "v_sub_f32 v47, v47, v7\n\t" \
   "v_pk_mul_f32 v[10:11], v[46:47], v[2:3] op_sel:[1,0] op_sel_hi:[1,1]\n\t" \
-  "global_store_dwordx4 v0, v[44:47], s[42:43] offset:3072\n\t" \
-  "global_load_dwordx4 v[44:47], v0, s[46:47] offset:3072\n\t" \
-  "s_add_u32 s42, s42, 8192\n\t" \
-  "s_addc_u32 s43, s43, 0\n\t" \
-  "s_add_u32 s46, s46, 8192\n\t" \
-  "s_addc_u32 s47, s47, 0\n\t" \
-  "s_waitcnt vmcnt(56)\n\t" \
-  "v_sub_f32 v48, v48, v10\n\t" \
-  "v_sub_f32 v48, v48, v9\n\t" \
-  "v_pk_mul_f32 v[4:5], v[48:49], v[2:3] op_sel:[0,0] op_sel_hi:[0,1]\n\t" \
-  "v_sub_f32 v49, v49, v4\n\t" \
-  "v_sub_f32 v49, v49, v11\n\t" \
-  "v_pk_mul_f32 v[6:7], v[48:49], v[2:3] op_sel:[1,0] op_sel_hi:[1,1]\n\t" \
-  "v_sub_f32 v50, v50, v6\n\t" \
-  "v_sub_f32 v50, v50, v5\n\t" \
-  "v_pk_mul_f32 v[8:9], v[50:51], v[2:3] op_sel:[0,0] op_sel_hi:[0,1]\n\t" \
-  "v_sub_f32 v51, v51, v8\n\t" \
-  "v_sub_f32 v51, v51, v7\n\t" \
-  "v_pk_mul_f32 v[10:11], v[50:51], v[2:3] op_sel:[1,0] op_sel_hi:[1,1]\n\t" \
-  "global_store_dwordx4 v0, v[48:51], s[42:43] offset:-4096\n\t" \
-  "global_load_dwordx4 v[48:51], v0, s[46:47] offset:-4096\n\t" \
-  "v_sub_f32 v52, v52, v10\n\t" \
-  "v_sub_f32 v52, v52, v9\n\t" \
-  "v_pk_mul_f32 v[4:5], v[52:53], v[2:3] op_sel:[0,0] op_sel_hi:[0,1]\n\t" \
-  "v_sub_f32 v53, v53, v4\n\t" \
-  "v_sub_f32 v53, v53, v11\n\t" \
-  "v_pk_mul_f32 v[6:7], v[52:53], v[2:3] op_sel:[1,0] op_sel_hi:[1,1]\n\t" \
-  "v_sub_f32 v54, v54, v6\n\t" \
-  "v_sub_f32 v54, v54, v5\n\t" \
-  "v_pk_mul_f32 v[8:9], v[54:55], v[2:3] op_sel:[0,0] op_sel_hi:[0,1]\n\t" \
-  "v_sub_f32 v55, v55, v8\n\t" \
-  "v_sub_f32 v55, v55, v7\n\t" \
-  "v_pk_mul_f32 v[10:11], v[54:55], v[2:3] op_sel:[1,0] op_sel_hi:[1,1]\n\t" \
-  "global_store_dwordx4 v0, v[52:55], s[42:43] offset:-3072\n\t" \
-  "global_load_dwordx4 v[52:55], v0, s[46:47] offset:-3072\n\t" \
-  "v_sub_f32 v56, v56, v10\n\t" \
-  "v_sub_f32 v56, v56, v9\n\t" \
-  "v_pk_mul_f32 v[4:5], v[56:57], v[2:3] op_sel:[0,0] op_sel_hi:[0,1]\n\t" \
-  "v_sub_f32 v57, v57, v4\n\t" \
-  "v_sub_f32 v57, v57, v11\n\t" \
-  "v_pk_mul_f32 v[6:7], v[56:57], v[2:3] op_sel:[1,0] op_sel_hi:[1,1]\n\t" \
-  "v_sub_f32 v58, v58, v6\n\t" \
-  "v_sub_f32 v58, v58, v5\n\t" \
-  "v_pk_mul_f32 v[8:9], v[58:59], v[2:3] op_sel:[0,0] op_sel_hi:[0,1]\n\t" \
-  "v_sub_f32 v59, v59, v8\n\t" \
-  "v_sub_f32 v59, v59, v7\n\t" \
-  "v_pk_mul_f32 v[10:11], v[58:59], v[2:3] op_sel:[1,0] op_sel_hi:[1,1]\n\t" \
-  "global_store_dwordx4 v0, v[56:59], s[42:43] offset:-2048\n\t" \
-  "global_load_dwordx4 v[56:59], v0, s[46:47] offset:-2048\n\t" \
-  "v_sub_f32 v60, v60, v10\n\t" \
-  "v_sub_f32 v60, v60, v9\n\t" \
-  "v_pk_mul_f32 v[4:5], v[60:61], v[2:3] op_sel:[0,0] op_sel_hi:[0,1]\n\t" \
-  "v_sub_f32 v61, v61, v4\n\t" \
-  "v_sub_f32 v61, v61, v11\n\t" \
-  "v_pk_mul_f32 v[6:7], v[60:61], v[2:3] op_sel:[1,0] op_sel_hi:[1,1]\n\t" \
-  "v_sub_f32 v62, v62, v6\n\t" \
-  "v_sub_f32 v62, v62, v5\n\t" \
-  "v_pk_mul_f32 v[8:9], v[62:63], v[2:3] op_sel:[0,0] op_sel_hi:[0,1]\n\t" \
-  "v_sub_f32 v63, v63, v8\n\t" \
-  "v_sub_f32 v63, v63, v7\n\t" \
-  "v_pk_mul_f32 v[10:11], v[62:63], v[2:3] op_sel:[1,0] op_sel_hi:[1,1]\n\t" \
-  "global_store_dwordx4 v0, v[60:63], s[42:43] offset:-1024\n\t" \
-  "global_load_dwordx4 v[60:63], v0, s[46:47] offset:-1024\n\t" \
-  "s_waitcnt vmcnt(56)\n\t" \
-  "v_sub_f32 v64, v64, v10\n\t" \
-  "v_sub_f32 v64, v64, v9\n\t" \
-  "v_pk_mul_f32 v[4:5], v[64:65], v[2:3] op_sel:[0,0] op_sel_hi:[0,1]\n\t" \
-  "v_sub_f32 v65, v65, v4\n\t" \
-  "v_sub_f32 v65, v65, v11\n\t" \
-  "v_pk_mul_f32 v[6:7], v[64:65], v[2:3] op_sel:[1,0] op_sel_hi:[1,1]\n\t" \
-  "v_sub_f32 v66, v66, v6\n\t" \
-  "v_sub_f32 v66, v66, v5\n\t" \
-  "v_pk_mul_f32 v[8:9], v[66:67], v[2:3] op_sel:[0,0] op_sel_hi:[0,1]\n\t" \
-  "v_sub_f32 v67, v67, v8\n\t" \
-  "v_sub_f32 v67, v67, v7\n\t" \
-  "v_pk_mul_f32 v[10:11], v[66:67], v[2:3] op_sel:[1,0] op_sel_hi:[1,1]\n\t" \
-  "global_store_dwordx4 v0, v[64:67], s[42:43] offset:0\n\t" \
-  "global_load_dwordx4 v[64:67], v0, s[46:47] offset:0\n\t" \
-  "v_sub_f32 v68, v68, v10\n\t" \
-  "v_sub_f32 v68, v68, v9\n\t" \
-  "v_pk_mul_f32 v[4:5], v[68:69], v[2:3] op_sel:[0,0] op_sel_hi:[0,1]\n\t" \
-  "v_sub_f32 v69, v69, v4\n\t" \
-  "v_sub_f32 v69, v69, v11\n\t" \
-  "v_pk_mul_f32 v[6:7], v[68:69], v[2:3] op_sel:[1,0] op_sel_hi:[1,1]\n\t" \
-  "v_sub_f32 v70, v70, v6\n\t" \
-  "v_sub_f32 v70, v70, v5\n\t" \
-  "v_pk_mul_f32 v[8:9], v[70:71], v[2:3] op_sel:[0,0] op_sel_hi:[0,1]\n\t" \
-  "v_sub_f32 v71, v71, v8\n\t" \
-  "v_sub_f32 v71, v71, v7\n\t" \
-  "v_pk_mul_f32 v[10:11], v[70:71], v[2:3] op_sel:[1,0] op_sel_hi:[1,1]\n\t" \
-  "global_store_dwordx4 v0, v[68:71], s[42:43] offset:1024\n\t" \
-  "global_load_dwordx4 v[68:71], v0, s[46:47] offset:1024\n\t" \
-  "v_sub_f32 v72, v72, v10\n\t" \
-  "v_sub_f32 v72, v72, v9\n\t" \
-  "v_pk_mul_f32 v[4:5], v[72:73], v[2:3] op_sel:[0,0] op_sel_hi:[0,1]\n\t" \
-  "v_sub_f32 v73, v73, v4\n\t" \
-  "v_sub_f32 v73, v73, v11\n\t" \
-  "v_pk_mul_f32 v[6:7], v[72:73], v[2:3] op_sel:[1,0] op_sel_hi:[1,1]\n\t" \
-  "v_sub_f32 v74, v74, v6\n\t" \
-  "v_sub_f32 v74, v74, v5\n\t" \
-  "v_pk_mul_f32 v[8:9], v[74:75], v[2:3] op_sel:[0,0] op_sel_hi:[0,1]\n\t" \
-  "v_sub_f32 v75, v75, v8\n\t" \
-  "v_sub_f32 v75, v75, v7\n\t" \
-  "v_pk_mul_f32 v[10:11], v[74:75], v[2:3] op_sel:[1,0] op_sel_hi:[1,1]\n\t" \
-  "global_store_dwordx4 v0, v[72:75], s[42:43] offset:2048\n\t" \
-  "global_load_dwordx4 v[72:75], v0, s[46:47] offset:2048\n\t" \
-  "v_sub_f32 v76, v76, v10\n\t" \
-  "v_sub_f32 v76, v76, v9\n\t" \
-  "v_pk_mul_f32 v[4:5], v[76:77], v[2:3] op_sel:[0,0] op_sel_hi:[0,1]\n\t" \
-  "v_sub_f32 v77, v77, v4\n\t" \
-  "v_sub_f32 v77, v77, v11\n\t" \
-  "v_pk_mul_f32 v[6:7], v[76:77], v[2:3] op_sel:[1,0] op_sel_hi:[1,1]\n\t" \
-  "v_sub_f32 v78, v78, v6\n\t" \
-  "v_sub_f32 v78, v78, v5\n\t" \
-  "v_pk_mul_f32 v[8:9], v[78:79], v[2:3] op_sel:[0,0] op_sel_hi:[0,1]\n\t" \
-  "v_sub_f32 v79, v79, v8\n\t" \
-  "v_sub_f32 v79, v79, v7\n\t" \
-  "v_pk_mul_f32 v[10:11], v[78:79], v[2:3] op_sel:[1,0] op_sel_hi:[1,1]\n\t" \
-  "global_store_dwordx4 v0, v[76:79], s[42:43] offset:3072\n\t" \
-  "global_load_dwordx4 v[76:79], v0, s[46:47] offset:3072\n\t" \
-  "s_add_u32 s42, s42, 8192\n\t" \
-  "s_addc_u32 s43, s43, 0\n\t" \
-  "s_add_u32 s46, s46, 8192\n\t" \
-  "s_addc_u32 s47, s47, 0\n\t" \
-  "s_waitcnt vmcnt(56)\n\t" \
-  "v_sub_f32 v80, v80, v10\n\t" \
-  "v_sub_f32 v80, v80, v9\n\t" \
-  "v_pk_mul_f32 v[4:5], v[80:81], v[2:3] op_sel:[0,0] op_sel_hi:[0,1]\n\t" \
-  "v_sub_f32 v81, v81, v4\n\t" \
-  "v_sub_f32 v81, v81, v11\n\t" \
-  "v_pk_mul_f32 v[6:7], v[80:81], v[2:3] op_sel:[1,0] op_sel_hi:[1,1]\n\t" \
-  "v_sub_f32 v82, v82, v6\n\t" \
-  "v_sub_f32 v82, v82, v5\n\t" \
-  "v_pk_mul_f32 v[8:9], v[82:83], v[2:3] op_sel:[0,0] op_sel_hi:[0,1]\n\t" \
-  "v_sub_f32 v83, v83, v8\n\t" \
-  "v_sub_f32 v83, v83, v7\n\t" \
-  "v_pk_mul_f32 v[10:11], v[82:83], v[2:3] op_sel:[1,0] op_sel_hi:[1,1]\n\t" \
-  "global_store_dwordx4 v0, v[80:83], s[42:43] offset:-4096\n\t" \
-  "global_load_dwordx4 v[80:83], v0, s[46:47] offset:-4096\n\t" \
-  "v_sub_f32 v84, v84, v10\n\t" \
-  "v_sub_f32 v84, v84, v9\n\t" \
-  "v_pk_mul_f32 v[4:5], v[84:85], v[2:3] op_sel:[0,0] op_sel_hi:[0,1]\n\t" \
-  "v_sub_f32 v85, v85, v4\n\t" \
-  "v_sub_f32 v85, v85, v11\n\t" \
-  "v_pk_mul_f32 v[6:7], v[84:85], v[2:3] op_sel:[1,0] op_sel_hi:[1,1]\n\t" \
-  "v_sub_f32 v86, v86, v6\n\t" \
-  "v_sub_f32 v86, v86, v5\n\t" \
-  "v_pk_mul_f32 v[8:9], v[86:87], v[2:3] op_sel:[0,0] op_sel_hi:[0,1]\n\t" \
-  "v_sub_f32 v87, v87, v8\n\t" \
-  "v_sub_f32 v87, v87, v7\n\t" \
-  "v_pk_mul_f32 v[10:11], v[86:87], v[2:3] op_sel:[1,0] op_sel_hi:[1,1]\n\t" \
-  "global_store_dwordx4 v0, v[84:87], s[42:43] offset:-3072\n\t" \
-  "global_load_dwordx4 v[84:87], v0, s[46:47] offset:-3072\n\t" \
-  "v_sub_f32 v88, v88, v10\n\t" \
-  "v_sub_f32 v88, v88, v9\n\t" \
-  "v_pk_mul_f32 v[4:5], v[88:89], v[2:3] op_sel:[0,0] op_sel_hi:[0,1]\n\t" \
-  "v_sub_f32 v89, v89, v4\n\t" \
-  "v_sub_f32 v89, v89, v11\n\t" \
-  "v_pk_mul_f32 v[6:7], v[88:89], v[2:3] op_sel:[1,0] op_sel_hi:[1,1]\n\t" \
-  "v_sub_f32 v90, v90, v6\n\t" \
-  "v_sub_f32 v90, v90, v5\n\t" \
-  "v_pk_mul_f32 v[8:9], v[90:91], v[2:3] op_sel:[0,0] op_sel_hi:[0,1]\n\t" \
-  "v_sub_f32 v91, v91, v8\n\t" \
-  "v_sub_f32 v91, v91, v7\n\t" \
-  "v_pk_mul_f32 v[10:11], v[90:91], v[2:3] op_sel:[1,0] op_sel_hi:[1,1]\n\t" \
-  "global_store_dwordx4 v0, v[88:91], s[42:43] offset:-2048\n\t" \
-  "global_load_dwordx4 v[88:91], v0, s[46:47] offset:-2048\n\t" \
-  "v_sub_f32 v92, v92, v10\n\t" \
-  "v_sub_f32 v92, v92, v9\n\t" \
-  "v_pk_mul_f32 v[4:5], v[92:93], v[2:3] op_sel:[0,0] op_sel_hi:[0,1]\n\t" \
-  "v_sub_f32 v93, v93, v4\n\t" \
-  "v_sub_f32 v93, v93, v11\n\t" \
-  "v_pk_mul_f32 v[6:7], v[92:93], v[2:3] op_sel:[1,0] op_sel_hi:[1,1]\n\t" \
-  "v_sub_f32 v94, v94, v6\n\t" \
-  "v_sub_f32 v94, v94, v5\n\t" \
-  "v_pk_mul_f32 v[8:9], v[94:95], v[2:3] op_sel:[0,0] op_sel_hi:[0,1]\n\t" \
-  "v_sub_f32 v95, v95, v8\n\t" \
-  "v_sub_f32 v95, v95, v7\n\t" \
-  "v_pk_mul_f32 v[10:11], v[94:95], v[2:3] op_sel:[1,0] op_sel_hi:[1,1]\n\t" \
-  "global_store_dwordx4 v0, v[92:95], s[42:43] offset:-1024\n\t" \
-  "global_load_dwordx4 v[92:95], v0, s[46:47] offset:-1024\n\t" \
-  "s_waitcnt vmcnt(56)\n\t" \
-  "v_sub_f32 v96, v96, v10\n\t" \
-  "v_sub_f32 v96, v96, v9\n\t" \
-  "v_pk_mul_f32 v[4:5], v[96:97], v[2:3] op_sel:[0,0] op_sel_hi:[0,1]\n\t" \
-  "v_sub_f32 v97, v97, v4\n\t" \
-  "v_sub_f32 v97, v97, v11\n\t" \
-  "v_pk_mul_f32 v[6:7], v[96:97], v[2:3] op_sel:[1,0] op_sel_hi:[1,1]\n\t" \
-  "v_sub_f32 v98, v98, v6\n\t" \
-  "v_sub_f32 v98, v98, v5\n\t" \
-  "v_pk_mul_f32 v[8:9], v[98:99], v[2:3] op_sel:[0,0] op_sel_hi:[0,1]\n\t" \
-  "v_sub_f32 v99, v99, v8\n\t" \
-  "v_sub_f32 v99, v99, v7\n\t" \
-  "v_pk_mul_f32 v[10:11], v[98:99], v[2:3] op_sel:[1,0] op_sel_hi:[1,1]\n\t" \
-  "global_store_dwordx4 v0, v[96:99], s[42:43] offset:0\n\t" \
-  "global_load_dwordx4 v[96:99], v0, s[46:47] offset:0\n\t" \
-  "v_sub_f32 v100, v100, v10\n\t" \
-  "v_sub_f32 v100, v100, v9\n\t" \
-  "v_pk_mul_f32 v[4:5], v[100:101], v[2:3] op_sel:[0,0] op_sel_hi:[0,1]\n\t" \
-  "v_sub_f32 v101, v101, v4\n\t" \
-  "v_sub_f32 v101, v101, v11\n\t" \
-  "v_pk_mul_f32 v[6:7], v[100:101], v[2:3] op_sel:[1,0] op_sel_hi:[1,1]\n\t" \
-  "v_sub_f32 v102, v102, v6\n\t" \
-  "v_sub_f32 v102, v102, v5\n\t" \
-  "v_pk_mul_f32 v[8:9], v[102:103], v[2:3] op_sel:[0,0] op_sel_hi:[0,1]\n\t" \
-  "v_sub_f32 v103, v103, v8\n\t" \
-  "v_sub_f32 v103, v103, v7\n\t" \
-  "v_pk_mul_f32 v[10:11], v[102:103], v[2:3] op_sel:[1,0] op_sel_hi:[1,1]\n\t" \
-  "global_store_dwordx4 v0, v[100:103], s[42:43] offset:1024\n\t" \
-  "global_load_dwordx4 v[100:103], v0, s[46:47] offset:1024\n\t" \
-  "v_sub_f32 v104, v104, v10\n\t" \
-  "v_sub_f32 v104, v104, v9\n\t" \
-  "v_pk_mul_f32 v[4:5], v[104:105], v[2:3] op_sel:[0,0] op_sel_hi:[0,1]\n\t" \
-  "v_sub_f32 v105, v105, v4\n\t" \
-  "v_sub_f32 v105, v105, v11\n\t" \
-  "v_pk_mul_f32 v[6:7], v[104:105], v[2:3] op_sel:[1,0] op_sel_hi:[1,1]\n\t" \
-  "v_sub_f32 v106, v106, v6\n\t" \
-  "v_sub_f32 v106, v106, v5\n\t" \
-  "v_pk_mul_f32 v[8:9], v[106:107], v[2:3] op_sel:[0,0] op_sel_hi:[0,1]\n\t" \
-  "v_sub_f32 v107, v107, v8\n\t" \
-  "v_sub_f32 v107, v107, v7\n\t" \
-  "v_pk_mul_f32 v[10:11], v[106:107], v[2:3] op_sel:[1,0] op_sel_hi:[1,1]\n\t" \
-  "global_store_dwordx4 v0, v[104:107], s[42:43] offset:2048\n\t" \
-  "global_load_dwordx4 v[104:107], v0, s[46:47] offset:2048\n\t" \
-  "v_sub_f32 v108, v108, v10\n\t" \
-  "v_sub_f32 v108, v108, v9\n\t" \
-  "v_pk_mul_f32 v[4:5], v[108:109], v[2:3] op_sel:[0,0] op_sel_hi:[0,1]\n\t" \
-  "v_sub_f32 v109, v109, v4\n\t" \
-  "v_sub_f32 v109, v109, v11\n\t" \
-  "v_pk_mul_f32 v[6:7], v[108:109], v[2:3] op_sel:[1,0] op_sel_hi:[1,1]\n\t" \
-  "v_sub_f32 v110, v110, v6\n\t" \
-  "v_sub_f32 v110, v110, v5\n\t" \
-  "v_pk_mul_f32 v[8:9], v[110:111], v[2:3] op_sel:[0,0] op_sel_hi:[0,1]\n\t" \
-  "v_sub_f32 v111, v111, v8\n\t" \
-  "v_sub_f32 v111, v111, v7\n\t" \
-  "v_pk_mul_f32 v[10:11], v[110:111], v[2:3] op_sel:[1,0] op_sel_hi:[1,1]\n\t" \
-  "global_store_dwordx4 v0, v[108:111], s[42:43] offset:3072\n\t" \
-  "global_load_dwordx4 v[108:111], v0, s[46:47] offset:3072\n\t" \
-  "s_add_u32 s42, s42, 8192\n\t" \
-  "s_addc_u32 s43, s43, 0\n\t" \
-  "s_add_u32 s46, s46, 8192\n\t" \
-  "s_addc_u32 s47, s47, 0\n\t" \
-  "s_waitcnt vmcnt(56)\n\t" \
-  "v_sub_f32 v112, v112, v10\n\t" \
-  "v_sub_f32 v112, v112, v9\n\t" \
-  "v_pk_mul_f32 v[4:5], v[112:113], v[2:3] op_sel:[0,0] op_sel_hi:[0,1]\n\t" \
-  "v_sub_f32 v113, v113, v4\n\t" \
-  "v_sub_f32 v113, v113, v11\n\t" \
-  "v_pk_mul_f32 v[6:7], v[112:113], v[2:3] op_sel:[1,0] op_sel_hi:[1,1]\n\t" \
-  "v_sub_f32 v114, v114, v6\n\t" \
-  "v_sub_f32 v114, v114, v5\n\t" \
-  "v_pk_mul_f32 v[8:9], v[114:115], v[2:3] op_sel:[0,0] op_sel_hi:[0,1]\n\t" \
-  "v_sub_f32 v115, v115, v8\n\t" \
-  "v_sub_f32 v115, v115, v7\n\t" \
-  "v_pk_mul_f32 v[10:11], v[114:115], v[2:3] op_sel:[1,0] op_sel_hi:[1,1]\n\t" \
-  "global_store_dwordx4 v0, v[112:115], s[42:43] offset:-4096\n\t" \
-  "global_load_dwordx4 v[112:115], v0, s[46:47] offset:-4096\n\t" \
-  "v_sub_f32 v116, v116, v10\n\t" \
-  "v_sub_f32 v116, v116, v9\n\t" \
-  "v_pk_mul_f32 v[4:5], v[116:117], v[2:3] op_sel:[0,0] op_sel_hi:[0,1]\n\t" \
-  "v_sub_f32 v117, v117, v4\n\t" \
-  "v_sub_f32 v117, v117, v11\n\t" \
-  "v_pk_mul_f32 v[6:7], v[116:117], v[2:3] op_sel:[1,0] op_sel_hi:[1,1]\n\t" \
-  "v_sub_f32 v118, v118, v6\n\t" \
-  "v_sub_f32 v118, v118, v5\n\t" \
-  "v_pk_mul_f32 v[8:9], v[118:119], v[2:3] op_sel:[0,0] op_sel_hi:[0,1]\n\t" \
-  "v_sub_f32 v119, v119, v8\n\t" \
-  "v_sub_f32 v119, v119, v7\n\t" \
-  "v_pk_mul_f32 v[10:11], v[118:119], v[2:3] op_sel:[1,0] op_sel_hi:[1,1]\n\t" \
-  "global_store_dwordx4 v0, v[116:119], s[42:43] offset:-3072\n\t" \
-  "global_load_dwordx4 v[116:119], v0, s[46:47] offset:-3072\n\t" \
-  "v_sub_f32 v120, v120, v10\n\t" \
-  "v_sub_f32 v120, v120, v9\n\t" \
-  "v_pk_mul_f32 v[4:5], v[120:121], v[2:3] op_sel:[0,0] op_sel_hi:[0,1]\n\t" \
-  "v_sub_f32 v121, v121, v4\n\t" \
-  "v_sub_f32 v121, v121, v11\n\t" \
-  "v_pk_mul_f32 v[6:7], v[120:121], v[2:3] op_sel:[1,0] op_sel_hi:[1,1]\n\t" \
-  "v_sub_f32 v122, v122, v6\n\t" \
-  "v_sub_f32 v122, v122, v5\n\t" \
-  "v_pk_mul_f32 v[8:9], v[122:123], v[2:3] op_sel:[0,0] op_sel_hi:[0,1]\n\t" \
-  "v_sub_f32 v123, v123, v8\n\t" \
-  "v_sub_f32 v123, v123, v7\n\t" \
-  "v_pk_mul_f32 v[10:11], v[122:123], v[2:3] op_sel:[1,0] op_sel_hi:[1,1]\n\t" \
-  "global_store_dwordx4 v0, v[120:123], s[42:43] offset:-2048\n\t" \
-  "global_load_dwordx4 v[120:123], v0, s[46:47] offset:-2048\n\t" \
-  "v_sub_f32 v124, v124, v10\n\t" \
-  "v_sub_f32 v124, v124, v9\n\t" \
-  "v_pk_mul_f32 v[4:5], v[124:125], v[2:3] op_sel:[0,0] op_sel_hi:[0,1]\n\t" \
-  "v_sub_f32 v125, v125, v4\n\t" \
-  "v_sub_f32 v125, v125, v11\n\t" \
-  "v_pk_mul_f32 v[6:7], v[124:125], v[2:3] op_sel:[1,0] op_sel_hi:[1,1]\n\t" \
-  "v_sub_f32 v126, v126, v6\n\t" \
-  "v_sub_f32 v126, v126, v5\n\t" \
-  "v_pk_mul_f32 v[8:9], v[126:127], v[2:3] op_sel:[0,0] op_sel_hi:[0,1]\n\t" \
-  "v_sub_f32 v127, v127, v8\n\t" \
-  "v_sub_f32 v127, v127, v7\n\t" \
-  "v_pk_mul_f32 v[10:11], v[126:127], v[2:3] op_sel:[1,0] op_sel_hi:[1,1]\n\t" \
-  "global_store_dwordx4 v0, v[124:127], s[42:43] offset:-1024\n\t" \
-  "global_load_dwordx4 v[124:127], v0, s[46:47] offset:-1024\n\t" \
-  "s_waitcnt vmcnt(56)\n\t" \
-  "v_sub_f32 v128, v128, v10\n\t" \
-  "v_sub_f32 v128, v128, v9\n\t" \
-  "v_pk_mul_f32 v[4:5], v[128:129], v[2:3] op_sel:[0,0] op_sel_hi:[0,1]\n\t" \
-  "v_sub_f32 v129, v129, v4\n\t" \
-  "v_sub_f32 v129, v129, v11\n\t" \
-  "v_pk_mul_f32 v[6:7], v[128:129], v[2:3] op_sel:[1,0] op_sel_hi:[1,1]\n\t" \
-  "v_sub_f32 v130, v130, v6\n\t" \
-  "v_sub_f32 v130, v130, v5\n\t" \
-  "v_pk_mul_f32 v[8:9], v[130:131], v[2:3] op_sel:[0,0] op_sel_hi:[0,1]\n\t" \
-  "v_sub_f32 v131, v131, v8\n\t" \
-  "v_sub_f32 v131, v131, v7\n\t" \
-  "v_pk_mul_f32 v[10:11], v[130:131], v[2:3] op_sel:[1,0] op_sel_hi:[1,1]\n\t" \
-  "global_store_dwordx4 v0, v[128:131], s[42:43] offset:0\n\t" \
-  "global_load_dwordx4 v[128:131], v0, s[46:47] offset:0\n\t" \
-  "v_sub_f32 v132, v132, v10\n\t" \
-  "v_sub_f32 v132, v132, v9\n\t" \
-  "v_pk_mul_f32 v[4:5], v[132:133], v[2:3] op_sel:[0,0] op_sel_hi:[0,1]\n\t" \
-  "v_sub_f32 v133, v133, v4\n\t" \
-  "v_sub_f32 v133, v133, v11\n\t" \
-  "v_pk_mul_f32 v[6:7], v[132:133], v[2:3] op_sel:[1,0] op_sel_hi:[1,1]\n\t" \
-  "v_sub_f32 v134, v134, v6\n\t" \
-  "v_sub_f32 v134, v134, v5\n\t" \
-  "v_pk_mul_f32 v[8:9], v[134:135], v[2:3] op_sel:[0,0] op_sel_hi:[0,1]\n\t" \
-  "v_sub_f32 v135, v135, v8\n\t" \
-  "v_sub_f32 v135, v135, v7\n\t" \
-  "v_pk_mul_f32 v[10:11], v[134:135], v[2:3] op_sel:[1,0] op_sel_hi:[1,1]\n\t" \
-  "global_store_dwordx4 v0, v[132:135], s[42:43] offset:1024\n\t" \
-  "global_load_dwordx4 v[132:135], v0, s[46:47] offset:1024\n\t" \
-  "v_sub_f32 v136, v136, v10\n\t" \
-  "v_sub_f32 v136, v136, v9\n\t" \
-  "v_pk_mul_f32 v[4:5], v[136:137], v[2:3] op_sel:[0,0] op_sel_hi:[0,1]\n\t" \
-  "v_sub_f32 v137, v137, v4\n\t" \
-  "v_sub_f32 v137, v137, v11\n\t" \
-  "v_pk_mul_f32 v[6:7], v[136:137], v[2:3] op_sel:[1,0] op_sel_hi:[1,1]\n\t" \
-  "v_sub_f32 v138, v138, v6\n\t" \
-  "v_sub_f32 v138, v138, v5\n\t" \
-  "v_pk_mul_f32 v[8:9], v[138:139], v[2:3] op_sel:[0,0] op_sel_hi:[0,1]\n\t" \
-  "v_sub_f32 v139, v139, v8\n\t" \
-  "v_sub_f32 v139, v139, v7\n\t" \
-  "v_pk_mul_f32 v[10:11], v[138:139], v[2:3] op_sel:[1,0] op_sel_hi:[1,1]\n\t" \
-  "global_store_dwordx4 v0, v[136:139], s[42:43] offset:2048\n\t" \
-  "global_load_dwordx4 v[136:139], v0, s[46:47] offset:2048\n\t" \
-  "v_sub_f32 v140, v140, v10\n\t" \
-  "v_sub_f32 v140, v140, v9\n\t" \
-  "v_pk_mul_f32 v[4:5], v[140:141], v[2:3] op_sel:[0,0] op_sel_hi:[0,1]\n\t" \
-  "v_sub_f32 v141, v141, v4\n\t" \
-  "v_sub_f32 v141, v141, v11\n\t" \
-  "v_pk_mul_f32 v[6:7], v[140:141], v[2:3] op_sel:[1,0] op_sel_hi:[1,1]\n\t" \
-  "v_sub_f32 v142, v142, v6\n\t" \
-  "v_sub_f32 v142, v142, v5\n\t" \
-  "v_pk_mul_f32 v[8:9], v[142:143], v[2:3] op_sel:[0,0] op_sel_hi:[0,1]\n\t" \
-  "v_sub_f32 v143, v143, v8\n\t" \
-  "v_sub_f32 v143, v143, v7\n\t" \
-  "v_pk_mul_f32 v[10:11], v[142:143], v[2:3] op_sel:[1,0] op_sel_hi:[1,1]\n\t" \
-  "global_store_dwordx4 v0, v[140:143], s[42:43] offset:3072\n\t" \
-  "global_load_dwordx4 v[140:143], v0, s[46:47] offset:3072\n\t" \
-  "s_add_u32 s42, s42, 8192\n\t" \
-  "s_addc_u32 s43, s43, 0\n\t" \
-  "s_add_u32 s46, s46, 8192\n\t" \
-  "s_addc_u32 s47, s47, 0\n\t" \
-  "s_add_u32 s40, s40, 32768\n\t" \
-  "s_addc_u32 s41, s41, 0\n\t" \
+  "ds_write_b128 v0, v[44:47] offset:1904\n\t" \
+  "ds_read_b128 v[44:47], v0 offset:4080\n\t" \
+  "s_waitcnt lgkmcnt(8)\n\t" \
+  "v_sub_f32 v16, v16, v10\n\t" \
+  "v_sub_f32 v16, v16, v9\n\t" \
+  "v_pk_mul_f32 v[4:5], v[16:17], v[2:3] op_sel:[0,0] op_sel_hi:[0,1]\n\t" \
+  "v_sub_f32 v17, v17, v4\n\t" \
+  "v_sub_f32 v17, v17, v11\n\t" \
+  "v_pk_mul_f32 v[6:7], v[16:17], v[2:3] op_sel:[1,0] op_sel_hi:[1,1]\n\t" \
+  "v_sub_f32 v18, v18, v6\n\t" \
+  "v_sub_f32 v18, v18, v5\n\t" \
+  "v_pk_mul_f32 v[8:9], v[18:19], v[2:3] op_sel:[0,0] op_sel_hi:[0,1]\n\t" \
+  "v_sub_f32 v19, v19, v8\n\t" \
+  "v_sub_f32 v19, v19, v7\n\t" \
+  "v_pk_mul_f32 v[10:11], v[18:19], v[2:3] op_sel:[1,0] op_sel_hi:[1,1]\n\t" \
+  "ds_write_b128 v0, v[16:19] offset:2176\n\t" \
+  "ds_read_b128 v[16:19], v1 offset:4352\n\t" \
+  "v_sub_f32 v20, v20, v10\n\t" \
+  "v_sub_f32 v20, v20, v9\n\t" \
+  "v_pk_mul_f32 v[4:5], v[20:21], v[2:3] op_sel:[0,0] op_sel_hi:[0,1]\n\t" \
+  "v_sub_f32 v21, v21, v4\n\t" \
+  "v_sub_f32 v21, v21, v11\n\t" \
+  "v_pk_mul_f32 v[6:7], v[20:21], v[2:3] op_sel:[1,0] op_sel_hi:[1,1]\n\t" \
+  "v_sub_f32 v22, v22, v6\n\t" \
+  "v_sub_f32 v22, v22, v5\n\t" \
+  "v_pk_mul_f32 v[8:9], v[22:23], v[2:3] op_sel:[0,0] op_sel_hi:[0,1]\n\t" \
+  "v_sub_f32 v23, v23, v8\n\t" \
+  "v_sub_f32 v23, v23, v7\n\t" \
+  "v_pk_mul_f32 v[10:11], v[22:23], v[2:3] op_sel:[1,0] op_sel_hi:[1,1]\n\t" \
+  "ds_write_b128 v0, v[20:23] offset:2448\n\t" \
+  "ds_read_b128 v[20:23], v1 offset:4624\n\t" \
+  "v_sub_f32 v24, v24, v10\n\t" \
+  "v_sub_f32 v24, v24, v9\n\t" \
+  "v_pk_mul_f32 v[4:5], v[24:25], v[2:3] op_sel:[0,0] op_sel_hi:[0,1]\n\t" \
+  "v_sub_f32 v25, v25, v4\n\t" \
+  "v_sub_f32 v25, v25, v11\n\t" \
+  "v_pk_mul_f32 v[6:7], v[24:25], v[2:3] op_sel:[1,0] op_sel_hi:[1,1]\n\t" \
+  "v_sub_f32 v26, v26, v6\n\t" \
+  "v_sub_f32 v26, v26, v5\n\t" \
+  "v_pk_mul_f32 v[8:9], v[26:27], v[2:3] op_sel:[0,0] op_sel_hi:[0,1]\n\t" \
+  "v_sub_f32 v27, v27, v8\n\t" \
+  "v_sub_f32 v27, v27, v7\n\t" \
+  "v_pk_mul_f32 v[10:11], v[26:27], v[2:3] op_sel:[1,0] op_sel_hi:[1,1]\n\t" \
+  "ds_write_b128 v0, v[24:27] offset:2720\n\t" \
+  "ds_read_b128 v[24:27], v1 offset:4896\n\t" \
+  "v_sub_f32 v28, v28, v10\n\t" \
+  "v_sub_f32 v28, v28, v9\n\t" \
+  "v_pk_mul_f32 v[4:5], v[28:29], v[2:3] op_sel:[0,0] op_sel_hi:[0,1]\n\t" \
+  "v_sub_f32 v29, v29, v4\n\t" \
+  "v_sub_f32 v29, v29, v11\n\t" \
+  "v_pk_mul_f32 v[6:7], v[28:29], v[2:3] op_sel:[1,0] op_sel_hi:[1,1]\n\t" \
+  "v_sub_f32 v30, v30, v6\n\t" \
+  "v_sub_f32 v30, v30, v5\n\t" \
+  "v_pk_mul_f32 v[8:9], v[30:31], v[2:3] op_sel:[0,0] op_sel_hi:[0,1]\n\t" \
+  "v_sub_f32 v31, v31, v8\n\t" \
+  "v_sub_f32 v31, v31, v7\n\t" \
+  "v_pk_mul_f32 v[10:11], v[30:31], v[2:3] op_sel:[1,0] op_sel_hi:[1,1]\n\t" \
+  "ds_write_b128 v0, v[28:31] offset:2992\n\t" \
+  "ds_read_b128 v[28:31], v1 offset:5168\n\t" \
+  "s_waitcnt lgkmcnt(8)\n\t" \
+  "v_sub_f32 v32, v32, v10\n\t" \
+  "v_sub_f32 v32, v32, v9\n\t" \
+  "v_pk_mul_f32 v[4:5], v[32:33], v[2:3] op_sel:[0,0] op_sel_hi:[0,1]\n\t" \
+  "v_sub_f32 v33, v33, v4\n\t" \
+  "v_sub_f32 v33, v33, v11\n\t" \
+  "v_pk_mul_f32 v[6:7], v[32:33], v[2:3] op_sel:[1,0] op_sel_hi:[1,1]\n\t" \
+  "v_sub_f32 v34, v34, v6\n\t" \
+  "v_sub_f32 v34, v34, v5\n\t" \
+  "v_pk_mul_f32 v[8:9], v[34:35], v[2:3] op_sel:[0,0] op_sel_hi:[0,1]\n\t" \
+  "v_sub_f32 v35, v35, v8\n\t" \
+  "v_sub_f32 v35, v35, v7\n\t" \
+  "v_pk_mul_f32 v[10:11], v[34:35], v[2:3] op_sel:[1,0] op_sel_hi:[1,1]\n\t" \
+  "ds_write_b128 v0, v[32:35] offset:3264\n\t" \
+  "ds_read_b128 v[32:35], v1 offset:5440\n\t" \
+  "v_sub_f32 v36, v36, v10\n\t" \
+  "v_sub_f32 v36, v36, v9\n\t" \
+  "v_pk_mul_f32 v[4:5], v[36:37], v[2:3] op_sel:[0,0] op_sel_hi:[0,1]\n\t" \
+  "v_sub_f32 v37, v37, v4\n\t" \
+  "v_sub_f32 v37, v37, v11\n\t" \
+  "v_pk_mul_f32 v[6:7], v[36:37], v[2:3] op_sel:[1,0] op_sel_hi:[1,1]\n\t" \
+  "v_sub_f32 v38, v38, v6\n\t" \
+  "v_sub_f32 v38, v38, v5\n\t" \
+  "v_pk_mul_f32 v[8:9], v[38:39], v[2:3] op_sel:[0,0] op_sel_hi:[0,1]\n\t" \
+  "v_sub_f32 v39, v39, v8\n\t" \
+  "v_sub_f32 v39, v39, v7\n\t" \
+  "v_pk_mul_f32 v[10:11], v[38:39], v[2:3] op_sel:[1,0] op_sel_hi:[1,1]\n\t" \
+  "ds_write_b128 v0, v[36:39] offset:3536\n\t" \
+  "ds_read_b128 v[36:39], v1 offset:5712\n\t" \
+  "v_sub_f32 v40, v40, v10\n\t" \
+  "v_sub_f32 v40, v40, v9\n\t" \
+  "v_pk_mul_f32 v[4:5], v[40:41], v[2:3] op_sel:[0,0] op_sel_hi:[0,1]\n\t" \
+  "v_sub_f32 v41, v41, v4\n\t" \
+  "v_sub_f32 v41, v41, v11\n\t" \
+  "v_pk_mul_f32 v[6:7], v[40:41], v[2:3] op_sel:[1,0] op_sel_hi:[1,1]\n\t" \
+  "v_sub_f32 v42, v42, v6\n\t" \
+  "v_sub_f32 v42, v42, v5\n\t" \
+  "v_pk_mul_f32 v[8:9], v[42:43], v[2:3] op_sel:[0,0] op_sel_hi:[0,1]\n\t" \
+  "v_sub_f32 v43, v43, v8\n\t" \
+  "v_sub_f32 v43, v43, v7\n\t" \
+  "v_pk_mul_f32 v[10:11], v[42:43], v[2:3] op_sel:[1,0] op_sel_hi:[1,1]\n\t" \
+  "ds_write_b128 v0, v[40:43] offset:3808\n\t" \
+  "ds_read_b128 v[40:43], v1 offset:5984\n\t" \
+  "v_sub_f32 v44, v44, v10\n\t" \
+  "v_sub_f32 v44, v44, v9\n\t" \
+  "v_pk_mul_f32 v[4:5], v[44:45], v[2:3] op_sel:[0,0] op_sel_hi:[0,1]\n\t" \
+  "v_sub_f32 v45, v45, v4\n\t" \
+  "v_sub_f32 v45, v45, v11\n\t" \
+  "v_pk_mul_f32 v[6:7], v[44:45], v[2:3] op_sel:[1,0] op_sel_hi:[1,1]\n\t" \
+  "v_sub_f32 v46, v46, v6\n\t" \
+  "v_sub_f32 v46, v46, v5\n\t" \
+  "v_pk_mul_f32 v[8:9], v[46:47], v[2:3] op_sel:[0,0] op_sel_hi:[0,1]\n\t" \
+  "v_sub_f32 v47, v47, v8\n\t" \
+  "v_sub_f32 v47, v47, v7\n\t" \
+  "v_pk_mul_f32 v[10:11], v[46:47], v[2:3] op_sel:[1,0] op_sel_hi:[1,1]\n\t" \
+  "ds_write_b128 v0, v[44:47] offset:4080\n\t" \
+  "ds_read_b128 v[44:47], v1 offset:6256\n\t" \
+  "v_add_u32 v0, 4352, v0\n\t" \
   "s_cmp_lg_u32 s44, 0\n\t" \
   "s_cbranch_scc1 Llfe_rot%=\n\t" \
-  "s_waitcnt vmcnt(0)\n\t" \
-  "v_mov_b32 %[y1], v143\n\t" \
-  "v_mov_b32 %[y2], v142\n\t" \
+  "s_waitcnt lgkmcnt(0)\n\t" \
+  "v_mov_b32 %[y1], v47\n\t" \
+  "v_mov_b32 %[y2], v46\n\t" \
   ""
 #define IAMF_LFE_ASM_CLOBBERS \
-  "v0", "v1", "v2", "v3", "v4", "v5", "v6", "v7", "v8", "v9", "v10", "v11", "v12", "v13", "v14", "v15", "v16", "v17", "v18", "v19", "v20", "v21", "v22", "v23", "v24", "v25", "v26", "v27", "v28", "v29", "v30", "v31", "v32", "v33", "v34", "v35", "v36", "v37", "v38", "v39", "v40", "v41", "v42", "v43", "v44", "v45", "v46", "v47", "v48", "v49", "v50", "v51", "v52", "v53", "v54", "v55", "v56", "v57", "v58", "v59", "v60", "v61", "v62", "v63", "v64", "v65", "v66", "v67", "v68", "v69", "v70", "v71", "v72", "v73", "v74", "v75", "v76", "v77", "v78", "v79", "v80", "v81", "v82", "v83", "v84", "v85", "v86", "v87", "v88", "v89", "v90", "v91", "v92", "v93", "v94", "v95", "v96", "v97", "v98", "v99", "v100", "v101", "v102", "v103", "v104", "v105", "v106", "v107", "v108", "v109", "v110", "v111", "v112", "v113", "v114", "v115", "v116", "v117", "v118", "v119", "v120", "v121", "v122", "v123", "v124", "v125", "v126", "v127", "v128", "v129", "v130", "v131", "v132", "v133", "v134", "v135", "v136", "v137", "v138", "v139", "v140", "v141", "v142", "v143", "s40", "s41", "s42", "s43", "s44", "s45", "s46", "s47", "scc", "memory"
+  "v0", "v1", "v2", "v3", "v4", "v5", "v6", "v7", "v8", "v9", "v10", "v11", "v12", "v13", "v14", "v15", "v16", "v17", "v18", "v19", "v20", "v21", "v22", "v23", "v24", "v25", "v26", "v27", "v28", "v29", "v30", "v31", "v32", "v33", "v34", "v35", "v36", "v37", "v38", "v39", "v40", "v41", "v42", "v43", "v44", "v45", "v46", "v47", "s44", "s45", "scc", "memory"
diff --git a/iac_amd/csrc/render_lfe.hpp b/iac_amd/csrc/render_lfe.hpp
--- a/iac_amd/csrc/render_lfe.hpp
+++ b/iac_amd/csrc/render_lfe.hpp
@@ -2,7 +2,14 @@
 
 #include "lfe_chain_asm.inc"
 
-constexpr int kLfeTileQ = 16;
+constexpr int kLfeSW = 16;
+constexpr int kLfeQ = 128;
+constexpr int kLfeRow = kLfeSW + 1;
+constexpr int kLfeHelpers = 512;
+constexpr int kLfeThreads = 64 + kLfeHelpers;
+constexpr int kLfePasses = kLfeQ * kLfeSW / kLfeHelpers;
+static_assert(64 % kLfeSW == 0 && (kLfeQ * kLfeSW) % kLfeHelpers == 0 && kLfeHelpers % 64 == 0, "tile shape");
+static_assert(kLfeQ % 16 == 0 && kLfeRow * 16 == IAMF_LFE_ROW_BYTES && kLfeQ % IAMF_LFE_RING == 0, "tile and asm loop");
 
 struct LfeParams {
   const float *in;
@@ -21,7 +28,13 @@
   return ((((int64_t)(s >> 6) * t4 + (k >> 2)) * 64 + (s & 63)) << 2) + (k & 3);
 }
 
-__device__ __forceinline__ float lfe_w_at(const LfeParams &p, int s, int k) {
+struct LfeSource {
+  const float *in, *pre_matrix, *state;
+  int64_t in_stream_stride, in_frame_stride;
+  int32_t pre_l, pre_m, frame_size, total;
+};
+
+__device__ __forceinline__ float lfe_w_at(const LfeSource &p, int s, int k) {
   const int f = k / p.frame_size, i = k - f * p.frame_size;
   const float *src = p.in + (int64_t)s * p.in_stream_stride + (int64_t)f * p.in_frame_stride + i;
   if (!p.pre_matrix) return src[0];
@@ -30,72 +43,107 @@
   return w;
 }
 
-__global__ __launch_bounds__(256) void lfe_ff_kernel(const LfeParams p) {
-  __shared__ float4 tile[kLfeTileQ * 65];
+struct LfeQuadIn {
+  float w[4], wm1, wm2;
+};
+__device__ __noinline__ LfeQuadIn lfe_fetch_general(const LfeSource p, int s, int k0) {
+  LfeQuadIn o;
+  o.wm1 = k0 >= 1 ? lfe_w_at(p, s, k0 - 1) : p.state[4 * s + 0];
+  o.wm2 = k0 >= 2 ? lfe_w_at(p, s, k0 - 2) : p.state[4 * s + 1];
+  for (int i = 0; i < 4; ++i) o.w[i] = k0 + i < p.total ? lfe_w_at(p, s, k0 + i) : 0.f;
+  return o;
+}
+
+struct LfeFetch {
+  float w[kLfePasses][4], wm1[kLfePasses], wm2[kLfePasses];
+};
+
+__device__ __forceinline__ void lfe_helper_slot(int h, int ps, int &ql, int &sl) {
+  const int idx = ps * kLfeHelpers + h, g = idx >> 4;
+  sl = g % kLfeSW;
+  ql = (g / kLfeSW) * 16 + (idx & 15);
+}
+
+__global__ __launch_bounds__(kLfeThreads) void lfe_chain_kernel(const LfeParams p) {
+  __shared__ float4 tiles[3][kLfeQ * kLfeRow];
+  __shared__ float wnext[kLfeSW][2];
   const int t = threadIdx.x;
-  const int q_base = blockIdx.x * kLfeTileQ, sb = blockIdx.y;
-#pragma unroll
-  for (int pass = 0; pass < 4; ++pass) {
-    const int q = t & 15, sl = (t >> 4) + 16 * pass;
-    const int s = sb * 64 + sl, k0 = 4 * (q_base + q);
-    float4 u = make_float4(0.f, 0.f, 0.f, 0.f);
-    if (s >= p.s_first && s < p.s_first + p.s_count && k0 < p.total) {
-      const float h1 = p.state[4 * s + 0], h2 = p.state[4 * s + 1];
-      float wm1, wm2, w[4], uu[4];
-      const bool quick = !p.pre_matrix && ((p.frame_size | p.in_stream_stride | p.in_frame_stride) & 3) == 0 &&
-                         (reinterpret_cast<uintptr_t>(p.in) & 15) == 0 && k0 + 4 <= p.total;
-      if (quick) {
-        const int f = k0 / p.frame_size, i0 = k0 - f * p.frame_size;
-        const float *src = p.in + (int64_t)s * p.in_stream_stride + (int64_t)f * p.in_frame_stride + i0;
-        const float4 q = *reinterpret_cast<const float4 *>(src);
-        w[0] = q.x, w[1] = q.y, w[2] = q.z, w[3] = q.w;
-        if (i0 >= 4) {
-          wm1 = src[-1];
-          wm2 = src[-2];
-        } else if (k0 == 0) {
-          wm1 = h1;
-          wm2 = h2;
+  const int s0 = blockIdx.x * kLfeSW;
+  const int nfull = p.total >> 2;
+  const int left = p.total - 4 * nfull;
+  const int ntiles = max(1, (p.t4 + kLfeQ - 1) / kLfeQ);
+  auto is_active = [&](int s) { return s >= p.s_first && s < p.s_first + p.s_count; };
+
+  const int h = t - 64;
+  const LfeSource src_of = {p.in, p.pre_matrix, p.state, p.in_stream_stride, p.in_frame_stride, p.pre_l, p.pre_m, p.frame_size, p.total};
+  LfeFetch f;
+  auto fetch = [&](int kt) {
+#pragma unroll
+    for (int ps = 0; ps < kLfePasses; ++ps) {
+      int ql, sl;
+      lfe_helper_slot(h, ps, ql, sl);
+      const int s = s0 + sl, k0 = 4 * (kt * kLfeQ + ql);
+      float wm1 = 0.f, wm2 = 0.f, w[4] = {0.f, 0.f, 0.f, 0.f};
+      if (is_active(s) && k0 < p.total) {
+        const bool quick = !p.pre_matrix && ((p.frame_size | p.in_stream_stride | p.in_frame_stride) & 3) == 0 &&
+                           (reinterpret_cast<uintptr_t>(p.in) & 15) == 0 && k0 + 4 <= p.total;
+        if (quick) {
+          const int fr = k0 / p.frame_size, i0 = k0 - fr * p.frame_size;
+          const float *src = p.in + (int64_t)s * p.in_stream_stride + (int64_t)fr * p.in_frame_stride + i0;
+          const float4 q = *reinterpret_cast<const float4 *>(src);
+          w[0] = q.x, w[1] = q.y, w[2] = q.z, w[3] = q.w;
+          const float *prv = p.in + (int64_t)s * p.in_stream_stride + (int64_t)(fr - 1) * p.in_frame_stride + p.frame_size;
+          const float *m1 = i0 >= 4 ? src - 1 : (k0 == 0 ? p.state + 4 * s + 0 : prv - 1);
+          const float *m2 = i0 >= 4 ? src - 2 : (k0 == 0 ? p.state + 4 * s + 1 : prv - 2);
+          wm1 = *m1;
+          wm2 = *m2;
         } else {
-          const float *prv = p.in + (int64_t)s * p.in_stream_stride + (int64_t)(f - 1) * p.in_frame_stride + p.frame_size;
-          wm1 = prv[-1];
-          wm2 = prv[-2];
+          const LfeQuadIn g = lfe_fetch_general(src_of, s, k0);
+          w[0] = g.w[0], w[1] = g.w[1], w[2] = g.w[2], w[3] = g.w[3], wm1 = g.wm1, wm2 = g.wm2;
         }
-      } else {
-        wm1 = k0 >= 1 ? lfe_w_at(p, s, k0 - 1) : h1;
-        wm2 = k0 >= 2 ? lfe_w_at(p, s, k0 - 2) : (k0 == 1 ? h1 : h2);
       }
+      f.wm1[ps] = wm1, f.wm2[ps] = wm2;
+#pragma unroll
+      for (int i = 0; i < 4; ++i) f.w[ps][i] = w[i];
+    }
+  };
+  auto put = [&](int kt, float4 *buf) {
+#pragma unroll
+    for (int ps = 0; ps < kLfePasses; ++ps) {
+      int ql, sl;
+      lfe_helper_slot(h, ps, ql, sl);
+      const int s = s0 + sl, k0 = 4 * (kt * kLfeQ + ql);
+      float uu[4];
 #pragma unroll
       for (int i = 0; i < 4; ++i) {
-        if (!quick) w[i] = k0 + i < p.total ? lfe_w_at(p, s, k0 + i) : 0.f;
-        const float a = i >= 1 ? w[i - 1] : wm1, b = i >= 2 ? w[i - 2] : (i == 1 ? wm1 : wm2);
-        uu[i] = (p.a1 * w[i] + p.a2 * a) + p.a3 * b;
+        const float a = i >= 1 ? f.w[ps][i - 1] : f.wm1[ps], b = i >= 2 ? f.w[ps][i - 2] : (i == 1 ? f.wm1[ps] : f.wm2[ps]);
+        uu[i] = (p.a1 * f.w[ps][i] + p.a2 * a) + p.a3 * b;
       }
-      u = make_float4(uu[0], uu[1], uu[2], uu[3]);
-      if (k0 + 4 >= p.total) {
+      if (is_active(s) && k0 < p.total && k0 + 4 >= p.total) {
         const int il = p.total - 1 - k0;
-        p.state_next[2 * s + 0] = w[il];
-        p.state_next[2 * s + 1] = il >= 1 ? w[il - 1] : wm1;
+        const float n1 = il == 3 ? f.w[ps][3] : (il == 2 ? f.w[ps][2] : (il == 1 ? f.w[ps][1] : f.w[ps][0]));
+        const float n2 = il == 3 ? f.w[ps][2] : (il == 2 ? f.w[ps][1] : (il == 1 ? f.w[ps][0] : f.wm1[ps]));
+        wnext[sl][0] = n1;
+        wnext[sl][1] = n2;
       }
-    }
-    tile[q * 65 + sl] = u;
-  }
-  __syncthreads();
-#pragma unroll
-  for (int pass = 0; pass < 4; ++pass) {
-    const int q = (t >> 6) + 4 * pass, sl = t & 63;
-    if (q_base + q < p.t4) p.u_t[((int64_t)sb * p.t4 + q_base + q) * 64 + sl] = tile[q * 65 + sl];
-  }
-}
-
-__global__ __launch_bounds__(64) void lfe_chain_kernel(const LfeParams p) {
-  const int lane = threadIdx.x, sb = blockIdx.x;
-  const int s = sb * 64 + lane;
-  const bool active = s >= p.s_first && s < p.s_first + p.s_count;
-  const int sc = active ? s : p.s_first;
-  float y1 = p.state[4 * sc + 2], y2 = p.state[4 * sc + 3];
+      buf[ql * kLfeRow + sl] = make_float4(uu[0], uu[1], uu[2], uu[3]);
+    }
+  };
+  auto drain = [&](int kt, const float4 *buf) {
+#pragma unroll
+    for (int ps = 0; ps < kLfePasses; ++ps) {
+      const int idx = ps * kLfeHelpers + h, sl = idx % kLfeSW, ql = idx / kLfeSW;
+      const int s = s0 + sl, q = kt * kLfeQ + ql;
+      if (q < p.t4 && is_active(s)) p.u_t[((int64_t)(s >> 6) * p.t4 + q) * 64 + (s & 63)] = buf[ql * kLfeRow + sl];
+    }
+  };
+
+  const int lane = t, sc = s0 + lane;
+  const bool chain = t < kLfeSW;
+  const bool active = chain && is_active(sc);
+  float y1 = 0.f, y2 = 0.f;
+  if (active) y1 = p.state[4 * sc + 2], y2 = p.state[4 * sc + 3];
   const float b1 = p.b1, b2 = p.b2;
-  float4 *row = p.u_t + (int64_t)sb * p.t4 * 64 + lane;
-  const int nfull = p.total >> 2;
   auto step4 = [&](const float4 u) {
     float4 o;
     o.x = (u.x - b1 * y1) - b2 * y2;
@@ -106,47 +154,62 @@
     y1 = o.w;
     return o;
   };
-  int q_done = 0;
-  {
-    const int nrot = nfull / IAMF_LFE_RING;
+  auto run_tile = [&](int kt, float4 *buf) {
+    float4 *row = buf + lane;
+    const int nq = min(max(nfull - kt * kLfeQ, 0), kLfeQ);
+    int q_done = 0;
+    const int nrot = nq / IAMF_LFE_RING;
     if (nrot > 0) {
-      const float4 *base = p.u_t + (int64_t)sb * p.t4 * 64;
-      const unsigned voff = (unsigned)lane * 16u;
+      const unsigned lds = (unsigned)(uintptr_t)(__attribute__((address_space(3))) float4 *)row;
       asm volatile(IAMF_LFE_ASM_BODY
                    : [y1] "+v"(y1), [y2] "+v"(y2)
-                   : [base] "s"(base), [nrot] "s"(nrot), [voff] "v"(voff), [b1] "v"(b1), [b2] "v"(b2)
+                   : [lds] "v"(lds), [nrot] "s"(nrot), [b1] "v"(b1), [b2] "v"(b2)
                    : IAMF_LFE_ASM_CLOBBERS);
       q_done = nrot * IAMF_LFE_RING;
     }
-  }
-  {
-    const int nrem = nfull - q_done;
-    float4 rem[IAMF_LFE_RING];
-#pragma unroll
-    for (int i = 0; i < IAMF_LFE_RING; ++i)
-      if (i < nrem) rem[i] = row[(int64_t)(q_done + i) * 64];
-#pragma unroll
-    for (int i = 0; i < IAMF_LFE_RING; ++i)
-      if (i < nrem) row[(int64_t)(q_done + i) * 64] = step4(rem[i]);
-  }
-  const int left = p.total - 4 * nfull;
-  if (left > 0) {
-    const float4 u = row[(int64_t)nfull * 64];
-    float4 o;
-    o.x = (u.x - b1 * y1) - b2 * y2;
-    o.y = (u.y - b1 * o.x) - b2 * y1;
-    o.z = (u.z - b1 * o.y) - b2 * o.x;
-    o.w = 0.f;
-    row[(int64_t)nfull * 64] = o;
-    const float r1 = left == 3 ? o.z : (left == 2 ? o.y : o.x);
-    const float r2 = left == 3 ? o.y : (left == 2 ? o.x : y1);
-    y2 = r2;
-    y1 = r1;
+    {
+      const int nrem = nq - q_done;
+      float4 rem[IAMF_LFE_RING];
+#pragma unroll
+      for (int i = 0; i < IAMF_LFE_RING; ++i)
+        if (i < nrem) rem[i] = row[(q_done + i) * kLfeRow];
+#pragma unroll
+      for (int i = 0; i < IAMF_LFE_RING; ++i)
+        if (i < nrem) row[(q_done + i) * kLfeRow] = step4(rem[i]);
+    }
+    if (left > 0 && nfull / kLfeQ == kt) {
+      const int ql = nfull - kt * kLfeQ;
+      const float4 u = row[ql * kLfeRow];
+      float4 o;
+      o.x = (u.x - b1 * y1) - b2 * y2;
+      o.y = (u.y - b1 * o.x) - b2 * y1;
+      o.z = (u.z - b1 * o.y) - b2 * o.x;
+      o.w = 0.f;
+      row[ql * kLfeRow] = o;
+      const float r1 = left == 3 ? o.z : (left == 2 ? o.y : o.x);
+      const float r2 = left == 3 ? o.y : (left == 2 ? o.x : y1);
+      y2 = r2;
+      y1 = r1;
+    }
+  };
+
+  for (int k = -2; k <= ntiles; ++k) {
+    if (t >= 64) {
+      if (k >= 1) drain(k - 1, tiles[(k + 2) % 3]);
+      if (k >= -1 && k + 1 < ntiles) put(k + 1, tiles[(k + 1) % 3]);
+      if (k + 2 < ntiles) fetch(k + 2);
+    } else if (chain && k >= 0 && k < ntiles) {
+      run_tile(k, tiles[k % 3]);
+    }
+    __syncthreads();
   }
   if (active) {
-    p.state[4 * s + 0] = p.state_next[2 * s + 0];
-    p.state[4 * s + 1] = p.state_next[2 * s + 1];
-    p.state[4 * s + 2] = y1;
-    p.state[4 * s + 3] = y2;
+    const float w1 = wnext[lane][0], w2 = wnext[lane][1];
+    p.state[4 * sc + 0] = w1;
+    p.state[4 * sc + 1] = w2;
+    p.state[4 * sc + 2] = y1;
+    p.state[4 * sc + 3] = y2;
+    p.state_next[2 * sc + 0] = w1;
+    p.state_next[2 * sc + 1] = w2;
   }
 }
```

Result: no change. 87280 (median of 2 runs) (+0.1%).
